# Stanford-ILIAD/PantheonRL

Measured on AMD Instinct MI355X. Metric: env-steps/sec (all agents) Overcooked-simple PPO self-play, higher is better.
Workload: dtype f32; 1 GPU; OvercookedMultiEnv-v0 layout=simple, PPO self-play (two independent PPO learners per GPU), synthetic (n_envs, n_steps, obs_dim) rollouts; n_envs=1024, n_steps=128, obs_dim=62, features=62, n_logits=6, batch_size=32768, n_epochs=10, agents_per_gpu=2, parallelism=2 agent(s) per gpu x1 gpu(s) = 2 learners (single process), launch_mode=graph, gemm_mode=2, action_masks=none, rollout=scripted, rollout_requested=scripted

## Files before the change

### include/pantheon_hip.h

```cpp
#ifndef PANTHEON_HIP_H
#define PANTHEON_HIP_H

#ifdef __cplusplus
extern "C" {
#endif

#define PH_ABI_VERSION 7
#define PH_HIDDEN 64
#define PH_MAX_COMP 256
#define PH_MAX_LOGITS 64
#define PH_MAX_BOX_ACT 16
#define PH_NSTAT 8
#define PH_MOD_MAX 8
#define PH_MAX_RANKS 16

#define PH_SPACE_BOX 0
#define PH_SPACE_DISCRETE 1

typedef struct ph_ctx ph_ctx;

typedef struct ph_space {
  int kind;
  int n;
  int nvec[PH_MAX_COMP];
// ... 8 lines not shown
  int D;
  int F;
  int A;
  int L;
  int P;
  int pi_W1, pi_b1, pi_W2, pi_b2, vf_W1, vf_b1, vf_W2, vf_b2, act_W, act_b, val_W, val_b;
} ph_layout;

typedef struct ph_rollout {
  int T, E;
  float *observations;
  float *actions;
  float *rewards;
  float *episode_starts;
  float *values;
  float *log_probs;
  float *advantages;
  float *returns;
} ph_rollout;

typedef struct ph_ppo_hyper {
  float learning_rate;
  float clip_range;
  float clip_range_vf;
  float ent_coef;
  float vf_coef;
  float max_grad_norm;
  float target_kl;
  int normalize_advantage;
  float adam_beta1, adam_beta2, adam_eps;
} ph_ppo_hyper;

typedef struct ph_opt_state {
  float *params;
  float *adam_m;
  float *adam_v;
  int *step;
} ph_opt_state;

int ph_abi_version(void);
const char *ph_last_error(void);
int ph_device_count(int *n_out );
int ph_ctx_create(int device, ph_ctx **out );
int ph_ctx_destroy(ph_ctx *ctx);
int ph_ctx_set_stream(ph_ctx *ctx, void *hip_stream );
int ph_ctx_sync(ph_ctx *ctx);
int ph_graph_begin(ph_ctx *ctx);
int ph_graph_end(ph_ctx *ctx, int *graph_id_out );
int ph_graph_launch(ph_ctx *ctx, int graph_id);
int ph_ctx_set_rng_epoch(ph_ctx *ctx, unsigned long long *epoch_dev );
int ph_rng_epoch_advance(ph_ctx *ctx);
int ph_debug_set_profile_buffer(ph_ctx *ctx, long long *stamps_dev);
int ph_debug_weight_image_mismatches(ph_ctx *ctx, const ph_spec *spec, const float *params, int *mismatches);
int ph_set_exclusive_device(ph_ctx *ctx, int exclusive);
int ph_ctx_step_errors(ph_ctx *ctx, unsigned int *count_out );
int ph_timer_start(ph_ctx *ctx);
int ph_timer_stop(ph_ctx *ctx, float *ms_out );

int ph_layout_of(const ph_spec *spec , ph_layout *out );
int ph_debug_split_tables(const ph_spec *spec, int *slab_map, int *image_map, int *eligible);
int ph_debug_split_oh_tables(const ph_spec *spec, int *slab_map, int *image_map, int *slab_len_out, int *image_elems_out,
                             int *eligible);

int ph_buffer_add(ph_ctx *ctx, const ph_spec *spec, const ph_rollout *rb, int pos, const float *obs ,
                  const float *actions , const float *episode_start ,
                  const float *values , const float *log_probs );
int ph_buffer_add_reward(ph_ctx *ctx, const ph_rollout *rb, int pos, const float *reward ,
                         const unsigned char *env_mask );
int ph_buffer_add_reward_const(ph_ctx *ctx, const ph_rollout *rb, int pos, float reward);
#define PH_JOINT_MATCH_BONUS 0
#define PH_JOINT_RPS 1
int ph_ctx_set_joint_reward_rule(ph_ctx *ctx, int rule);

int ph_buffer_add_reward_joint(ph_ctx *ctx, const ph_rollout *rb, int pos, const float *base_reward ,
                               const int *joint_actions, int n_seats, int seat, const int *partner_seat ,
                               float bonus);
int ph_roundrobin_env_step(ph_ctx *ctx, const int *joint_actions, int *partnerid, const float *base_reward,
                           const float *done, float *reward_out, int *alt_action_out, float *next_block, int block_ld,
                           int n_partners, float bonus, int n);
typedef struct ph_rr_link {
  int n_partners, rank;
  int n, block_ld;
  void *area[PH_MAX_RANKS];
  unsigned long long *error;
  unsigned long long timeout_cycles;
} ph_rr_link;
typedef struct ph_rr_ego {
  const ph_spec *spec;
  const float *params;
  const float *obs_seq;
  const float *base_reward_seq;
  const float *done_seq;
  float *blocks;
  int *partnerid;
  float *rewards;
  int *alt_actions;
  int *partner_trace;
  const float *episode_start0;
  unsigned long long seed, counter0;
  float *values, *log_probs;
  const ph_rollout *rb;
  float bonus;
} ph_rr_ego;
typedef struct ph_rr_partner {
  const ph_spec *spec;
  const float *params;
// ... 444 lines not shown
```

### pantheonrl_amd/_native.py

```python
from __future__ import annotations

import ctypes as C
import os
from typing import Optional, Sequence

PH_HIDDEN = 64
PH_MAX_COMP = 256
PH_MAX_LOGITS = 64
PH_MAX_BOX_ACT = 16
PH_NSTAT = 8
PH_SPACE_BOX = 0
PH_SPACE_DISCRETE = 1
STAT_NAMES = ("policy_loss", "value_loss", "entropy_loss", "clip_fraction", "approx_kl", "loss", "grad_norm", "applied")

_HERE = os.path.dirname(os.path.abspath(__file__))
LIB_PATH = os.environ.get("PANTHEON_HIP_LIB") or os.path.join(_HERE, "csrc", "libpantheon_hip.so")


class NativeError(RuntimeError):
    """Raised for any non-zero status from the C ABI (message from ph_last_error)."""


class PhSpace(C.Structure):
    _fields_ = [("kind", C.c_int), ("n", C.c_int), ("nvec", C.c_int * PH_MAX_COMP)]
# ... 160 lines not shown
                ("alt_values", C.c_void_p), ("alt_log_probs", C.c_void_p), ("alt_pos", C.c_void_p),
                ("alt_boundary", C.c_void_p), ("alt_term", C.c_void_p), ("alt_open", C.c_void_p), ("alt_acted", C.c_void_p),
                ("alt_seed", C.c_ulonglong),
                ("obs_ego", C.c_void_p), ("obs_alt", C.c_void_p), ("episodes", C.c_void_p),
                ("es_alt", C.c_void_p), ("running", C.c_void_p), ("can", C.c_void_p), ("done", C.c_void_p)]


PH_BLOCK_STATE_WORDS = 12

PH_MAX_POOL = 8
PH_POOL_LEARNER, PH_POOL_FROZEN, PH_POOL_SCRIPTED = 0, 1, 2
POOL_RESAMPLE = {"robin": 0, "random": 1}


class PhPoolMember(C.Structure):
    _fields_ = [("kind", C.c_int), ("params", C.c_void_p), ("rb", C.POINTER(PhRollout)), ("pos", C.c_void_p),
                ("boundary", C.c_void_p), ("term", C.c_void_p), ("open", C.c_void_p), ("values", C.c_void_p),
                ("log_probs", C.c_void_p), ("seed", C.c_ulonglong)]


class PhLiarPool(C.Structure):
    _fields_ = [("n", C.c_int), ("spec", C.POINTER(PhSpec)),
                ("hands", C.c_void_p), ("history", C.c_void_p), ("nmoves", C.c_void_p), ("ego_first", C.c_void_p),
                ("dice_seed", C.c_ulonglong), ("probegostart", C.c_float),
                ("ego_params", C.c_void_p), ("ego_rb", C.POINTER(PhRollout)), ("ego_actions", C.c_void_p),
                ("ego_values", C.c_void_p), ("ego_log_probs", C.c_void_p), ("ego_episode_start", C.c_void_p),
                ("ego_seed", C.c_ulonglong),
                ("members", C.POINTER(PhPoolMember)), ("n_members", C.c_int), ("partnerid", C.c_void_p),
                ("resample", C.c_int), ("pool_seed", C.c_ulonglong),
                ("alt_actions", C.c_void_p), ("alt_acted", C.c_void_p),
                ("obs_ego", C.c_void_p), ("obs_alt", C.c_void_p), ("episodes", C.c_void_p),
                ("obs_next", C.c_void_p), ("rew1", C.c_void_p), ("rew2", C.c_void_p), ("es_alt", C.c_void_p),
                ("done1", C.c_void_p), ("done2", C.c_void_p), ("running", C.c_void_p), ("can", C.c_void_p),
                ("alt_opens", C.c_void_p), ("ego_opens", C.c_void_p), ("done", C.c_void_p)]

SIGNATURES = {
    "ph_abi_version": [],
    "ph_roundrobin_env_step": [_vp, _vp, _vp, _vp, _vp, _vp, _vp, _vp, _i, _i, C.c_float, _i],
    "ph_last_error": [],
    "ph_device_count": [C.POINTER(_i)],
    "ph_ctx_create": [_i, C.POINTER(_vp)],
    "ph_ctx_destroy": [_vp],
    "ph_ctx_set_stream": [_vp, _vp],
    "ph_ctx_sync": [_vp],
    "ph_graph_begin": [_vp],
    "ph_graph_end": [_vp, C.POINTER(_i)],
    "ph_graph_launch": [_vp, _i],
    "ph_ctx_set_rng_epoch": [_vp, _vp],
    "ph_rng_epoch_advance": [_vp],
    "ph_debug_set_profile_buffer": [_vp, _vp],
    "ph_set_exclusive_device": [_vp, _i],
    "ph_ctx_step_errors": [_vp, C.POINTER(C.c_uint)],
    "ph_debug_weight_image_mismatches": [_vp, C.POINTER(PhSpec), _vp, C.POINTER(C.c_int)],
    "ph_timer_start": [_vp],
    "ph_timer_stop": [_vp, C.POINTER(C.c_float)],
    "ph_layout_of": [C.POINTER(PhSpec), C.POINTER(PhLayout)],
    "ph_debug_split_tables": [C.POINTER(PhSpec), C.POINTER(C.c_int), C.POINTER(C.c_int), C.POINTER(C.c_int)],
    "ph_debug_split_oh_tables": [C.POINTER(PhSpec), _vp, _vp, C.POINTER(_i), C.POINTER(_i), C.POINTER(_i)],
    "ph_buffer_add": [_vp, C.POINTER(PhSpec), C.POINTER(PhRollout), _i, _vp, _vp, _vp, _vp, _vp],
    "ph_buffer_add_reward": [_vp, C.POINTER(PhRollout), _i, _vp, _vp],
    "ph_buffer_add_reward_joint": [_vp, C.POINTER(PhRollout), _i, _vp, _vp, _i, _i, _vp, C.c_float],
    "ph_buffer_reset": [_vp, C.POINTER(PhSpec), C.POINTER(PhRollout)],
    "ph_gae": [_vp, C.POINTER(PhRollout), _vp, _vp, _d, _d, _i],
    "ph_policy_forward": [_vp, C.POINTER(PhSpec), _vp, _vp, _i, _vp, _vp, _vp, _ull, _ull, _i, _vp, _vp, _vp, _vp, _vp,
                          _vp, C.POINTER(PhRollout), _i, _vp, _vp, _i],
    "ph_ctx_set_joint_reward_rule": [_vp, _i],
    "ph_adapmult_layout_of": [C.POINTER(PhSpec), _i, _vp],
    "ph_adapmult_forward": [_vp, C.POINTER(PhSpec), _i, _vp, _vp, _i, _vp, _vp, _vp, _ull, _ull, _i, _vp, _vp, _vp, _vp, _vp,
                            _vp, C.POINTER(PhRollout), _i, _vp],
    "ph_adapmult_minibatch_grad": [_vp, C.POINTER(PhSpec), _i, _vp, C.POINTER(PhRollout), C.POINTER(PhPpoHyper), _vp, _i, _vp, _vp,
                                   _vp],
    "ph_adapmult_train": [_vp, C.POINTER(PhSpec), _i, C.POINTER(PhOptState), C.POINTER(PhRollout), C.POINTER(PhPpoHyper), _i, _i,
                          _vp, _ull, _vp, _vp],
    "ph_policy_act_host": [_vp, C.POINTER(PhSpec), _vp, _vp, _i, _vp, _ull, _ull, _i, _vp, _vp, _vp, C.POINTER(PhRollout), _i, _i],
    "ph_buffer_add_reward_const": [_vp, C.POINTER(PhRollout), _i, C.c_float],
    "ph_policy_step_multi": [_vp, _i, C.POINTER(PhStepCall)],
    "ph_policy_forward_ragged": [_vp, C.POINTER(PhSpec), _vp, _vp, _vp, _ull, _ull, _i, _vp, _vp, _vp, C.POINTER(PhRollout),
                                 _vp, _vp, _vp],
    "ph_buffer_add_reward_ragged": [_vp, C.POINTER(PhRollout), _vp, _vp, _vp],
    "ph_ragged_advance": [_vp, C.POINTER(PhRollout), _vp, _vp],
    "ph_buffer_compact_columns": [_vp, C.POINTER(PhSpec), C.POINTER(PhRollout), C.POINTER(PhRollout), _vp, _i],
    "ph_fix_illegal_actions": [_vp, _vp, _vp, _i, _i],
    "ph_rps_step": [_vp, _vp, _vp, _vp, _vp, _i],
    "ph_liar_step": [_vp, _vp, _vp, _vp, _vp, _vp, _vp, _vp, _vp, _vp, _i],
    "ph_liar_reset": [_vp, _vp, _vp, _vp, _vp, _vp, _ull, _ull, C.c_float, _i],
    "ph_liar_obs": [_vp, _vp, _vp, _vp, _vp, _vp, _vp, _i],
    "ph_liar_selfplay_step": [_vp, C.POINTER(PhLiarSelfPlay), _i, _ull, _i],
    "ph_liar_selfplay_rollout": [_vp, C.POINTER(PhLiarSelfPlay), _i, _i, _ull],
    "ph_pool_forward": [_vp, C.POINTER(PhSpec), C.POINTER(PhPoolMember), _i, _vp, _vp, _vp, _ull, _vp, _vp, _i],
    "ph_liar_default_actions": [_vp, _vp, _vp, _vp, _i],
    "ph_liar_pool_step": [_vp, C.POINTER(PhLiarPool), _i, _ull, _i],
    "ph_block_reset": [_vp, _i, _vp, _vp, _ull, _ull, _i],
    "ph_block_step": [_vp, _i, _vp, _vp, _i, _vp, _vp, _vp, _vp, _i],
    "ph_block_obs": [_vp, _i, _vp, _i, _vp, _vp, _i],
    "ph_block_selfplay_step": [_vp, C.POINTER(PhBlockSelfPlay), _i, _ull],
    "ph_block_replay_host": [_i, _i, _i, _vp, _vp, _vp, _vp, _vp, _vp, _vp, _i, _ull, _ull, _i],
    "ph_framestack_push": [_vp, _vp, _vp, _vp, _vp, _i, _i, _i],
    "ph_scripted_rollout": [_vp, C.POINTER(PhSpec), _vp, _vp, _vp, _vp, _i, _i, _vp, _ull, _ull, _vp, _vp, _vp,
                            C.POINTER(PhRollout), _i, _i],
    "ph_ppo_train": [_vp, C.POINTER(PhSpec), C.POINTER(PhOptState), C.POINTER(PhRollout), C.POINTER(PhPpoHyper), _i, _i,
                     _vp, _ull, _vp, _i],
    "ph_ppo_train_multi": [C.POINTER(PhTrainCall), _i],
    "ph_comm_unique_id": [_vp],
    "ph_comm_init": [_vp, _vp, _i, _i],
    "ph_comm_destroy": [_vp],
    "ph_all_gather_i32": [_vp, _vp, _vp, _i],
# ... 114 lines not shown
def make_arch(widths: Sequence[int]) -> PhArch:
    a = PhArch()
    a.n_layers = len(widths)
    for i, w in enumerate(list(widths)[:PH_ARCH_MAX_LAYERS]):
        a.width[i] = int(w)
    return a


def arch_layout_of(spec: PhSpec, arch: PhArch) -> PhArchLayout:
    lay = PhArchLayout()
    check(load().ph_arch_layout_of(C.byref(spec), C.byref(arch), C.byref(lay)))
    return lay


def arch_lds_bytes(spec: PhSpec, arch: PhArch):
    g, r, f = C.c_int(0), C.c_int(0), C.c_int(0)
    check(load().ph_arch_lds_bytes(C.byref(spec), C.byref(arch), C.byref(g), C.byref(r), C.byref(f)))
    return g.value, r.value, f.value


def adapmult_layout_of(spec: PhSpec, context_size: int) -> PhAdapMultLayout:
    lay = PhAdapMultLayout()
    check(load().ph_adapmult_layout_of(C.byref(spec), int(context_size), C.byref(lay)))
    return lay


def ptr(t) -> Optional[int]:
    if t is None:
        return None
    return t.data_ptr()


class Context:

    def __init__(self, device_index: int = 0):
        self.lib = load()
        h = C.c_void_p()
        check(self.lib.ph_ctx_create(int(device_index), C.byref(h)))
        self.handle = h
        self.device_index = int(device_index)
        self.exclusive_hint = False

    def set_stream(self, raw_stream: int) -> None:
        if raw_stream != getattr(self, "_bound_stream", None):
            check(self.lib.ph_ctx_set_stream(self.handle, C.c_void_p(raw_stream)))
            self._bound_stream = raw_stream

    def sync(self) -> None:
        check(self.lib.ph_ctx_sync(self.handle))

    def set_joint_reward_rule(self, rule: str) -> None:
        check(self.lib.ph_ctx_set_joint_reward_rule(self.handle, {"match": 0, "rps": 1}[rule]))

    def step_errors(self) -> int:
        n = C.c_uint(0)
        check(self.lib.ph_ctx_step_errors(self.handle, C.byref(n)))
        return int(n.value)

    def set_exclusive_device(self, exclusive: bool) -> None:
        check(self.lib.ph_set_exclusive_device(self.handle, int(bool(exclusive))))
        self.exclusive_hint = bool(exclusive)

    def close(self) -> None:
        if getattr(self, "handle", None):
            self.lib.ph_ctx_destroy(self.handle)
            self.handle = None

    def __del__(self):
        try:
            self.close()
        except Exception:
            pass


def feistel_indices(n: int, perm_seed: int, epoch: int, start: int = 0, count: Optional[int] = None):
    import numpy as np
    count = n - start if count is None else count
    out = (C.c_int * count)()
    check(load().ph_feistel_indices(int(n), int(perm_seed), int(epoch), int(start), int(count), out))
    return np.frombuffer(out, dtype=np.int32).copy()


def block_replay_host(variant: int, state=None, tokens=None, alt_actions=None, n: Optional[int] = None, seed: Optional[int] = None,
                      counter: int = 0, max_draws: int = -1):
    import numpy as np
    reset = state is None
    if reset:
        state = np.zeros((int(n), PH_BLOCK_STATE_WORDS), np.int32)
    state = np.ascontiguousarray(state, np.int32).copy()
    n = state.shape[0]
    R = 0 if tokens is None else int(np.shape(tokens)[0])
    De, Da, A = ((98, 50, 3) if variant == 1 else (40, 21, 2))
    tok = np.ascontiguousarray(np.zeros((0, n)) if tokens is None else tokens, np.int32).reshape(R, n)
    act = np.ascontiguousarray(np.zeros((0, n, A)) if alt_actions is None else alt_actions, np.int32).reshape(R, n, A)
    alt_obs, ego_obs = np.zeros((R, n, Da), np.float32), np.zeros((R, n, De), np.float32)
    rew, done = np.zeros((R, n, 2), np.float32), np.zeros((R, n), np.uint8)
    p = lambda a: a.ctypes.data_as(C.c_void_p)
    check(load().ph_block_replay_host(int(variant), n, R, p(state), p(tok), p(act), p(alt_obs), p(rew), p(done), p(ego_obs),
                                      int(reset), int(seed or 0), int(counter), int(max_draws)))
    return dict(state=state, alt_obs=alt_obs, rewards=rew, done=done, ego_obs=ego_obs)
```

### pantheonrl_amd/csrc/ph_abi.hip

```cpp
#include <dlfcn.h>
#include <hip/hip_runtime.h>
#include <rccl/rccl.h>

#include <atomic>
#include <chrono>
#include <cmath>
#include <cstdio>
#include <cstdint>
#include <cstring>
#include <mutex>
#include <string>
#include <vector>

#include "ph_launch.h"
#include "ph_block.h"
#include "ph_arch.h"
#include "ph_pool.h"

namespace ph {

namespace {
struct LdsGrant {
  const void* kernel;
  int device;
// ... 62 lines not shown
struct SpecCache {
  ph_spec spec;
  int* obs_off = nullptr;
  int* act_off = nullptr;
  int* slab_map = nullptr;
  int* slab_map_split = nullptr;
  int* wimage_map = nullptr;
  int split_kind = 0;
  int slab_len_split = 0;
  int wimage_elems = 0;
  int id = 0;
};

}

struct ph_ctx {
  int device = 0;
  hipStream_t stream = nullptr;
  float* slabs = nullptr;
  size_t slabs_cap = 0;
  float* statpart = nullptr;
  size_t statpart_cap = 0;
  float* grad = nullptr;
  size_t grad_cap = 0;
  float* blocksq = nullptr;
  size_t blocksq_cap = 0;
  float* advstats = nullptr;
  size_t advstats_cap = 0;
  float* act_stage_host = nullptr;
  float* act_stage_dev = nullptr;
  size_t act_stage_cap = 0;
  unsigned int* act_done_host = nullptr;
  unsigned int* act_done_dev = nullptr;
  unsigned int act_seq = 0;
  unsigned int* fwd_host_done = nullptr;
  int joint_reward_rule = 0;
  int wimage_zeroed_for = 0;
  size_t wimage_cap = 0;
  bool exclusive = false;
  unsigned short* wimage = nullptr;
  double* advpart = nullptr;
  size_t advpart_cap = 0;
  int* perm_idx = nullptr;
  size_t perm_idx_cap = 0;
  int* perm_phys = nullptr;
  size_t perm_phys_cap = 0;
  uint4* ximg = nullptr;
  size_t ximg_cap = 0;
  uint4* rec_pi = nullptr;
  uint4* rec_vf = nullptr;
  size_t rec_cap = 0;
  uint4* rowrec = nullptr;
  size_t rowrec_cap = 0;
  unsigned long long* step_words = nullptr;
  size_t step_words_cap = 0;
  unsigned int* step_gen = nullptr;
  float* am_buf = nullptr;
  size_t am_buf_cap = 0;
  float* adap_extra = nullptr;
  size_t adap_extra_cap = 0;
  float* adap_loss = nullptr;
  size_t adap_loss_cap = 0;
  float* scalars = nullptr;
  int* stop_flag = nullptr;
  std::vector<SpecCache> specs;
  std::vector<hipGraphExec_t> graphs;
  bool capturing = false;
  hipEvent_t ev0 = nullptr, ev1 = nullptr;
  ph_p2p* p2p_dev = nullptr;
  ph_p2p p2p_host;
  bool p2p_valid = false;
  void* comm = nullptr;
  int comm_world = 1, comm_rank = 0;
  hipEvent_t ev_grad = nullptr;
  int num_cu = 256;
  int exchange_blocks_per_cu = 0;
  unsigned long long* rng_epoch = nullptr;
  ph::PoolMemberDev* pool_dev = nullptr;
  ph::PoolMemberDev pool_host[PH_MAX_POOL];
  int pool_count = 0;
  int* pool_order = nullptr;
  size_t pool_order_cap = 0;
  int* pool_tiles = nullptr;
  size_t pool_tiles_cap = 0;
  long long* prof = nullptr;
  struct ModWs {
    float* act = nullptr;
    size_t act_cap = 0;
    int* maps = nullptr;
    ph_spec spec;
    ph_modular mod;
    bool maps_valid = false;
    float* kl_sum = nullptr;
    int* scratch = nullptr;
  } mw;
};

namespace {

struct DevGuard {
  int prev = -1;
  bool switched = false;
  explicit DevGuard(const ph_ctx* ctx) {
    if (!ctx) return;
    if (hipGetDevice(&prev) == hipSuccess && prev != ctx->device) switched = hipSetDevice(ctx->device) == hipSuccess;
  }
  ~DevGuard() {
    if (switched) (void)hipSetDevice(prev);
  }
  DevGuard(const DevGuard&) = delete;
  DevGuard& operator=(const DevGuard&) = delete;
};

template <typename T>
int ensure(const ph_ctx* ctx, T*& p, size_t& cap, size_t n) {
  if (n <= cap) return 0;
  if (ctx->capturing) return fail("workspace would grow inside graph capture: run the same call once outside capture first");
  if (p) (void)hipFree(p);
  p = nullptr;
  cap = 0;
  hipError_t e = hipMalloc((void**)&p, n * sizeof(T));
  if (e != hipSuccess) return fail_hip("hipMalloc(workspace)", e);
  cap = n;
  return 0;
}

int check_space(const ph_space& s, const char* name) {
  if (s.kind != PH_SPACE_BOX && s.kind != PH_SPACE_DISCRETE) return fail(std::string(name) + ": unknown space kind");
  if (s.n <= 0) return fail(std::string(name) + ": empty space");
  if (s.kind == PH_SPACE_DISCRETE) {
    if (s.n > PH_MAX_COMP) return fail(std::string(name) + ": too many components");
    for (int i = 0; i < s.n; ++i)
      if (s.nvec[i] <= 0) return fail(std::string(name) + ": nvec entries must be positive");
  }
  return 0;
}

int layout_of(const ph_spec* spec, ph_layout* o) {
  if (!spec || !o) return fail("null spec/layout");
  if (check_space(spec->obs, "observation space")) return 1;
  if (check_space(spec->act, "action space")) return 1;
  const bool gauss = spec->act.kind == PH_SPACE_BOX;
  if (gauss && spec->act.n > PH_MAX_BOX_ACT) return fail("Box action spaces: at most PH_MAX_BOX_ACT dimensions");
  o->D = spec->obs.n;
  o->F = 0;
  if (spec->obs.kind == PH_SPACE_BOX) o->F = spec->obs.n;
  else
    for (int i = 0; i < spec->obs.n; ++i) o->F += spec->obs.nvec[i];
  o->A = spec->act.n;
  o->L = 0;
  if (gauss) o->L = spec->act.n;
  else
    for (int i = 0; i < spec->act.n; ++i) o->L += spec->act.nvec[i];
  if (o->L > PH_MAX_LOGITS) return fail("too many logits (PH_MAX_LOGITS)");
  const int H = PH_HIDDEN;
  int off = 0;
  o->pi_W1 = off; off += o->F * H;
// ... 239 lines not shown
  ad.nblk = ph::reduce_blocks(slab_len);
  ad.P = P;
  ad.step = opt->step;
  ad.scalars = ctx->scalars;
  ad.stop_flag = ctx->stop_flag;
  ad.lr = hp->learning_rate;
  ad.beta1 = hp->adam_beta1;
  ad.beta2 = hp->adam_beta2;
  ad.eps = hp->adam_eps;
  ad.max_norm = hp->max_grad_norm;
  ad.stats_out = stats_out;
  ad.wimage = wimage;
  ad.wimage_map = wimage_map;
  return ad;
}

int check_train_call(const char* who, const ph_ctx* ctx, const ph_opt_state* opt, const ph_ppo_hyper* hp, int n_epochs,
                     int batch_size, bool aligned = true) {
  const std::string w(who);
  if (!ctx) return fail("null ctx");
  if (!opt || !opt->params || !opt->adam_m || !opt->adam_v || !opt->step) return fail(w + ": null optimizer state");
  if (aligned && (uintptr_t)opt->params % 16 != 0) return fail(w + ": params must be 16-byte aligned");
  if (!hp) return fail(w + ": null hyper-parameters");
  if (n_epochs <= 0 || batch_size <= 0) return fail(w + ": n_epochs and batch_size must be positive");
  return 0;
}
int check_minibatch_call(const char* who, const ph_ctx* ctx, const float* params, const ph_rollout* rb, const ph_ppo_hyper* hp,
                         const int* indices, int nb, const float* grad_out, bool aligned = true) {
  const std::string w(who);
  if (!ctx) return fail("null ctx");
  if (!params || !hp || !indices || !grad_out) return fail(w + ": null argument");
  if (aligned && (uintptr_t)params % 16 != 0) return fail(w + ": params must be 16-byte aligned");
  if (check_rb(rb)) return 1;
  if (nb <= 0) return fail(w + ": nb must be positive");
  return 0;
}

template <typename F>
int time_reps(ph_ctx* ctx, int warm, int reps, F&& fn, float* avg_ms) {
  for (int i = 0; i < warm; ++i)
    if (fn(i)) return 1;
  PH_HIP(hipEventRecord(ctx->ev0, ctx->stream));
  for (int i = 0; i < reps; ++i)
    if (fn(i)) return 1;
  PH_HIP(hipEventRecord(ctx->ev1, ctx->stream));
  PH_HIP(hipEventSynchronize(ctx->ev1));
  float ms = 0.f;
  PH_HIP(hipEventElapsedTime(&ms, ctx->ev0, ctx->ev1));
  *avg_ms = ms / (float)reps;
  return 0;
}
int hip_rc(hipError_t e, const char* what) { return e == hipSuccess ? 0 : fail_hip(what, e); }

}

extern "C" {

int ph_abi_version(void) { return PH_ABI_VERSION; }
const char* ph_last_error(void) { return g_err.c_str(); }

int ph_device_count(int* n_out) {
  if (!n_out) return fail("null n_out");
  int n = 0;
  hipError_t e = hipGetDeviceCount(&n);
  if (e != hipSuccess) {
    *n_out = 0;
    return fail_hip("hipGetDeviceCount", e);
  }
  *n_out = n;
  return 0;
}

int ph_ctx_create(int device, ph_ctx** out) {
  if (!out) return fail("null out");
  *out = nullptr;
  int n = 0;
  hipError_t e = hipGetDeviceCount(&n);
  if (e != hipSuccess || n <= 0) return fail("no HIP device visible: the PantheonRL MI355X engine has no CPU fallback");
  if (device < 0 || device >= n) return fail("device index out of range");
  ph_ctx probe;
  probe.device = device;
  DevGuard dev_guard(&probe);
  hipDeviceProp_t prop;
  PH_HIP(hipGetDeviceProperties(&prop, device));
  if (std::strncmp(prop.gcnArchName, "gfx950", 6) != 0)
    return fail(std::string("device is ") + prop.gcnArchName + ", this library is built for gfx950 (MI355X) only");
  ph_ctx* c = new ph_ctx();
  c->device = device;
  c->num_cu = prop.multiProcessorCount;
  if (hipMalloc((void**)&c->scalars, 4 * sizeof(float)) != hipSuccess ||
      hipMalloc((void**)&c->stop_flag, sizeof(int)) != hipSuccess) {
    delete c;
    return fail("hipMalloc(ctx scalars) failed");
  }
  (void)hipMemset(c->scalars, 0, 4 * sizeof(float));
  (void)hipMemset(c->stop_flag, 0, sizeof(int));
  (void)hipEventCreate(&c->ev0);
  (void)hipEventCreate(&c->ev1);
  *out = c;
  return 0;
}

int ph_ctx_destroy(ph_ctx* ctx) {
  DevGuard dev_guard(ctx);
  if (!ctx) return 0;
  (void)hipStreamSynchronize(ctx->stream);
  for (auto g : ctx->graphs)
    if (g) (void)hipGraphExecDestroy(g);
  for (auto& s : ctx->specs) {
    if (s.obs_off) (void)hipFree(s.obs_off);
    if (s.slab_map) (void)hipFree(s.slab_map);
    if (s.slab_map_split) (void)hipFree(s.slab_map_split);
    if (s.wimage_map) (void)hipFree(s.wimage_map);
    if (s.act_off) (void)hipFree(s.act_off);
  }
  void* ptrs[] = {ctx->wimage, ctx->mw.act, ctx->mw.maps, ctx->mw.kl_sum, ctx->mw.scratch, ctx->advpart, ctx->p2p_dev, ctx->slabs, ctx->statpart, ctx->grad, ctx->blocksq, ctx->advstats, ctx->perm_idx, ctx->perm_phys, ctx->ximg, ctx->rec_pi, ctx->rec_vf, ctx->rowrec, ctx->step_words, ctx->step_gen, ctx->scalars, ctx->stop_flag,
                  ctx->adap_extra, ctx->adap_loss, ctx->am_buf, ctx->pool_dev, ctx->pool_order, ctx->pool_tiles};
  for (void* p : ptrs)
    if (p) (void)hipFree(p);
  if (ctx->act_stage_host) (void)hipHostFree(ctx->act_stage_host);
  if (ctx->act_done_host) (void)hipHostFree(ctx->act_done_host);
  if (ctx->ev0) (void)hipEventDestroy(ctx->ev0);
  if (ctx->ev1) (void)hipEventDestroy(ctx->ev1);
  if (ctx->ev_grad) (void)hipEventDestroy(ctx->ev_grad);
  (void)ph_comm_destroy(ctx);
  delete ctx;
  return 0;
}

int ph_ctx_set_joint_reward_rule(ph_ctx* ctx, int rule) {
  if (!ctx) return fail("null ctx");
  if (rule != PH_JOINT_MATCH_BONUS && rule != PH_JOINT_RPS) return fail("ph_ctx_set_joint_reward_rule: unknown rule");
  ctx->joint_reward_rule = rule;
  return 0;
}

int ph_ctx_set_stream(ph_ctx* ctx, void* hip_stream) {
  DevGuard dev_guard(ctx);
  if (!ctx) return fail("null ctx");
  ctx->stream = (hipStream_t)hip_stream;
  return 0;
}

int ph_ctx_sync(ph_ctx* ctx) {
  DevGuard dev_guard(ctx);
  if (!ctx) return fail("null ctx");
  PH_HIP(hipStreamSynchronize(ctx->stream));
  return 0;
}

int ph_graph_begin(ph_ctx* ctx) {
  DevGuard dev_guard(ctx);
  if (!ctx) return fail("null ctx");
  if (ctx->capturing) return fail("already capturing");
  if (ctx->stream == nullptr) return fail("graph capture needs a non-default stream (ph_ctx_set_stream)");
  PH_HIP(hipStreamBeginCapture(ctx->stream, hipStreamCaptureModeRelaxed));
  ctx->capturing = true;
  return 0;
}

int ph_graph_end(ph_ctx* ctx, int* graph_id_out) {
  DevGuard dev_guard(ctx);
  if (!ctx || !graph_id_out) return fail("null ctx/graph_id_out");
  if (!ctx->capturing) return fail("not capturing");
  ctx->capturing = false;
  hipGraph_t g = nullptr;
  PH_HIP(hipStreamEndCapture(ctx->stream, &g));
  hipGraphExec_t ge = nullptr;
  hipError_t e = hipGraphInstantiate(&ge, g, nullptr, nullptr, 0);
  (void)hipGraphDestroy(g);
  if (e != hipSuccess) return fail_hip("hipGraphInstantiate", e);
  ctx->graphs.push_back(ge);
  *graph_id_out = (int)ctx->graphs.size() - 1;
  return 0;
}

int ph_graph_launch(ph_ctx* ctx, int graph_id) {
  DevGuard dev_guard(ctx);
  if (!ctx) return fail("null ctx");
  if (graph_id < 0 || graph_id >= (int)ctx->graphs.size()) return fail("bad graph id");
  PH_HIP(hipGraphLaunch(ctx->graphs[graph_id], ctx->stream));
  return 0;
}

int ph_ctx_set_rng_epoch(ph_ctx* ctx, unsigned long long* epoch_dev) {
  DevGuard dev_guard(ctx);
  if (!ctx) return fail("null ctx");
  ctx->rng_epoch = epoch_dev;
  return 0;
}
int ph_rng_epoch_advance(ph_ctx* ctx) {
  DevGuard dev_guard(ctx);
  if (!ctx) return fail("null ctx");
  if (!ctx->rng_epoch) return fail("ph_rng_epoch_advance: no epoch word attached");
  PH_HIP(ph::launch_epoch_advance(ctx->rng_epoch, ctx->stream));
  return 0;
}

int ph_debug_set_profile_buffer(ph_ctx* ctx, long long* stamps_dev) {
  DevGuard dev_guard(ctx);
  if (!ctx) return fail("null ctx");
  ctx->prof = stamps_dev;
  return 0;
}

int ph_debug_weight_image_mismatches(ph_ctx* ctx, const ph_spec* spec, const float* params, int* mismatches_host) {
  DevGuard dev_guard(ctx);
  if (!ctx || !params || !mismatches_host) return fail("ph_debug_weight_image_mismatches: null argument");
  ph::NetDims nd;
  if (resolve(ctx, spec, &nd)) return 1;
  *mismatches_host = -1;
  if (!ctx->wimage || !nd.wimage_map) return 0;
  int* d = nullptr;
  PH_HIP(hipMalloc((void**)&d, sizeof(int)));
  PH_HIP(hipMemsetAsync(d, 0, sizeof(int), ctx->stream));
  PH_HIP(ph::launch_weight_image_check(params, ctx->wimage, nd.wimage_map, nd.lay.P, d, ctx->stream));
  PH_HIP(hipMemcpyAsync(mismatches_host, d, sizeof(int), hipMemcpyDeviceToHost, ctx->stream));
  PH_HIP(hipStreamSynchronize(ctx->stream));
  (void)hipFree(d);
  return 0;
}

int ph_set_exclusive_device(ph_ctx* ctx, int exclusive) {
  if (!ctx) return fail("null ctx");
  ctx->exclusive = exclusive != 0;
  return 0;
}

int ph_ctx_step_errors(ph_ctx* ctx, unsigned int* count_out) {
  DevGuard dev_guard(ctx);
  if (!ctx || !count_out) return fail("ph_ctx_step_errors: null argument");
  *count_out = 0u;
  if (!ctx->step_gen) return 0;
  PH_HIP(hipMemcpyAsync(count_out, ctx->step_gen + 1, sizeof(unsigned int), hipMemcpyDeviceToHost, ctx->stream));
  PH_HIP(hipStreamSynchronize(ctx->stream));
  return 0;
}

int ph_timer_start(ph_ctx* ctx) {
  DevGuard dev_guard(ctx);
  if (!ctx) return fail("null ctx");
  PH_HIP(hipEventRecord(ctx->ev0, ctx->stream));
  return 0;
}
int ph_timer_stop(ph_ctx* ctx, float* ms_out) {
  DevGuard dev_guard(ctx);
  if (!ctx || !ms_out) return fail("null ctx/ms_out");
  PH_HIP(hipEventRecord(ctx->ev1, ctx->stream));
  PH_HIP(hipEventSynchronize(ctx->ev1));
  PH_HIP(hipEventElapsedTime(ms_out, ctx->ev0, ctx->ev1));
  return 0;
}

int ph_layout_of(const ph_spec* spec, ph_layout* out) { return layout_of(spec, out); }

int ph_debug_split_tables(const ph_spec* spec, int* slab_map , int* image_map , int* eligible) {
  if (!spec || !slab_map || !image_map || !eligible) return fail("ph_debug_split_tables: null argument");
  ph_layout lay;
  if (layout_of(spec, &lay)) return 1;
  ph::NetDims probe;
  std::memset(&probe, 0, sizeof(probe));
  probe.lay = lay;
  probe.nchunk = (lay.F + PH_HIDDEN - 1) / PH_HIDDEN;
  probe.A = lay.A;
  probe.L = lay.L;
  probe.F = lay.F;
  probe.obs_kind = spec->obs.kind;
  *eligible = ph::grad_split_eligible(probe) ? 1 : 0;
  if (!*eligible) return 0;
  ph::grad_slab_map_split(lay, slab_map, ph::grad_fast_fold(probe));
  ph::grad_weight_image_map(lay, ph::grad_fast_fold(probe), image_map);
  return 0;
}

int ph_debug_split_oh_tables(const ph_spec* spec, int* slab_map, int* image_map , int* slab_len_out, int* image_elems_out,
                             int* eligible) {
  if (!spec || !slab_len_out || !image_elems_out || !eligible) return fail("ph_debug_split_oh_tables: null argument");
  ph_layout lay;
  if (layout_of(spec, &lay)) return 1;
  ph::NetDims probe;
  std::memset(&probe, 0, sizeof(probe));
  probe.lay = lay;
  probe.nchunk = (lay.F + PH_HIDDEN - 1) / PH_HIDDEN;
  probe.A = lay.A;
  probe.L = lay.L;
  probe.F = lay.F;
  probe.D = lay.D;
  probe.obs_kind = spec->obs.kind;
  *eligible = ph::grad_split_oh_eligible(probe) ? 1 : 0;
  if (!*eligible) return 0;
  *slab_len_out = ph::grad_split_oh_slab_len(probe);
  *image_elems_out = ph::grad_split_oh_wimage_elems(probe);
  if (slab_map) ph::grad_slab_map_split_oh(lay, probe.nchunk, slab_map);
  if (image_map) ph::grad_weight_image_map_oh(lay, probe.nchunk, image_map);
  return 0;
}

int ph_buffer_add(ph_ctx* ctx, const ph_spec* spec, const ph_rollout* rb, int pos, const float* obs,
                  const float* actions, const float* episode_start, const float* values, const float* log_probs) {
  DevGuard dev_guard(ctx);
  if (!ctx) return fail("null ctx");
  ph_layout lay;
  if (layout_of(spec, &lay) || check_rb(rb)) return 1;
  if (pos < 0 || pos >= rb->T) return fail("ph_buffer_add: pos out of range (buffer full?)");
  if (!obs || !actions || !episode_start || !values || !log_probs) return fail("ph_buffer_add: null input");
  const size_t E = rb->E, row = (size_t)pos * E;
  PH_HIP(ph::launch_buffer_add(rb->observations + row * lay.D, rb->actions + row * lay.A, rb->rewards + row,
                               rb->episode_starts + row, rb->values + row, rb->log_probs + row, obs, actions,
                               episode_start, values, log_probs, rb->E, lay.D, lay.A, ctx->stream));
  return 0;
}

int ph_buffer_compact_columns(ph_ctx* ctx, const ph_spec* spec, const ph_rollout* src, const ph_rollout* dst,
                              const int* cols, int n) {
  DevGuard dev_guard(ctx);
  if (!ctx) return fail("null ctx");
  ph_layout lay;
  if (layout_of(spec, &lay) || check_rb(src) || check_rb(dst)) return 1;
  if (!cols || n <= 0 || n > src->E) return fail("ph_buffer_compact_columns: bad column list");
  if (dst->T != src->T || dst->E != n) return fail("ph_buffer_compact_columns: destination must be (T, n)");
  PH_HIP(ph::launch_buffer_compact(*src, *dst, cols, n, lay.D, lay.A, ctx->stream));
  return 0;
}

int ph_buffer_add_reward(ph_ctx* ctx, const ph_rollout* rb, int pos, const float* reward,
                         const unsigned char* env_mask) {
  DevGuard dev_guard(ctx);
  if (!ctx) return fail("null ctx");
  if (check_rb(rb)) return 1;
  if (pos < 0 || pos >= rb->T) return fail("ph_buffer_add_reward: pos out of range");
  if (!reward) return fail("ph_buffer_add_reward: null reward");
  PH_HIP(ph::launch_reward_add(rb->rewards + (size_t)pos * rb->E, reward, env_mask, rb->E, ctx->stream));
  return 0;
}

int ph_buffer_add_reward_const(ph_ctx* ctx, const ph_rollout* rb, int pos, float reward) {
  DevGuard dev_guard(ctx);
  if (!ctx) return fail("null ctx");
  if (check_rb(rb)) return 1;
  if (pos < 0 || pos >= rb->T) return fail("ph_buffer_add_reward_const: pos out of range");
  PH_HIP(ph::launch_reward_add_const(rb->rewards + (size_t)pos * rb->E, reward, rb->E, ctx->stream));
  return 0;
}

int ph_buffer_add_reward_joint(ph_ctx* ctx, const ph_rollout* rb, int pos, const float* base_reward,
                               const int* joint_actions, int n_seats, int seat, const int* partner_seat, float bonus) {
  DevGuard dev_guard(ctx);
  if (!ctx) return fail("null ctx");
  if (check_rb(rb)) return 1;
  if (pos < 0 || pos >= rb->T) return fail("ph_buffer_add_reward_joint: pos out of range");
  if (!base_reward || !joint_actions || !partner_seat) return fail("ph_buffer_add_reward_joint: null argument");
  if (n_seats <= 0 || seat < 0 || seat >= n_seats) return fail("ph_buffer_add_reward_joint: bad seat");
  PH_HIP(ph::launch_reward_add_joint(rb->rewards + (size_t)pos * rb->E, base_reward, joint_actions, rb->E, n_seats, seat,
                                     partner_seat, bonus, ctx->joint_reward_rule, ctx->stream));
  return 0;
}

int ph_roundrobin_env_step(ph_ctx* ctx, const int* joint_actions, int* partnerid, const float* base_reward, const float* done,
                           float* reward_out, int* alt_action_out, float* next_block, int block_ld, int n_partners,
                           float bonus, int n) {
  DevGuard dev_guard(ctx);
  if (!ctx) return fail("null ctx");
  if (!joint_actions || !partnerid || !base_reward || !done || !reward_out)
    return fail("ph_roundrobin_env_step: null argument");
  if (n <= 0 || n_partners <= 0) return fail("ph_roundrobin_env_step: bad sizes");
  if (next_block && block_ld < 3) return fail("ph_roundrobin_env_step: routing block rows need >= 3 header columns");
  PH_HIP(ph::launch_roundrobin_env_step(joint_actions, partnerid, base_reward, done, reward_out, alt_action_out, next_block,
                                        block_ld, n_partners, bonus, n, ctx->stream));
  return 0;
}

namespace {
constexpr size_t RR_STAMP_BYTES = 64 * sizeof(unsigned long long);
size_t rr_slot_bytes(int n_partners, int n, int block_ld) {
  const size_t blk = (size_t)n * (block_ld + 1) * sizeof(float), act = (size_t)(n_partners + 1) * n * sizeof(int);
  return ((blk > act ? blk : act) + 255) / 256 * 256;
}
int check_rr_link(const ph_rr_link* l) {
  if (!l) return fail("null ph_rr_link");
  if (l->n_partners < 1 || l->n_partners + 1 > PH_MAX_RANKS) return fail("ph_rr_link: n_partners out of range");
  if (l->rank < 0 || l->rank > l->n_partners || l->n <= 0 || l->block_ld <= 3) return fail("ph_rr_link: bad rank / n / block_ld");
  if (!l->error) return fail("ph_rr_link: error word required");
  for (int r = 0; r <= l->n_partners; ++r)
    if (!l->area[r]) return fail("ph_rr_link: unmapped peer area");
  return 0;
}
unsigned long long* rr_stamps(const ph_rr_link* l, int rank) { return (unsigned long long*)l->area[rank]; }
unsigned int* rr_arrive(const ph_rr_link* l) { return (unsigned int*)((unsigned long long*)l->area[0] + 32); }
char* rr_slot(const ph_rr_link* l, int rank, int parity) {
  return (char*)l->area[rank] + RR_STAMP_BYTES + (size_t)parity * rr_slot_bytes(l->n_partners, l->n, l->block_ld);
}
}

int ph_rr_area_bytes(int n_partners, int n, int block_ld, size_t* bytes_out) {
  if (!bytes_out || n_partners < 1 || n <= 0 || block_ld <= 3) return fail("ph_rr_area_bytes: bad argument");
  *bytes_out = RR_STAMP_BYTES + 2 * rr_slot_bytes(n_partners, n, block_ld);
  return 0;
}

int ph_roundrobin_ego_iteration(ph_ctx* ctx, const ph_rr_link* link, const ph_rr_ego* ego, int T, unsigned long long iteration) {
// ... 63 lines not shown
    return fail("ph_roundrobin_partner_iteration: null argument");
  if (check_rb(pa->rb)) return 1;
  if (pa->rb->E != link->n) return fail("ph_roundrobin_partner_iteration: the rollout buffer must have one column per environment");
  const int n = link->n, k = link->rank - 1;
  for (int t = 0; t < T; ++t) {
    const unsigned long long want = iteration * (unsigned long long)T + (unsigned long long)t + 1ull;
    ph::RRPartnerStep st;
    std::memset(&st, 0, sizeof(st));
    st.block_stamp = rr_stamps(link, link->rank);
    st.act_stamp = rr_stamps(link, 0) + 1 + k;
    st.want = want;
    st.timeout = link->timeout_cycles;
    st.error = link->error;
    st.block = (const float*)rr_slot(link, link->rank, t & 1);
    st.block_ld = link->block_ld;
    st.n = n;
    st.T = pa->rb->T;
    st.k = k;
    st.rewards = pa->rb->rewards;
    st.pos = pa->pos;
    st.boundary = pa->boundary;
    st.term = pa->term;
    st.open = pa->open;
    st.prev_mask = pa->prev_mask;
    st.can = pa->can_scratch;
    st.es = pa->es_scratch;
    st.actions = pa->actions;
    st.act_dst = (int*)rr_slot(link, 0, t & 1) + (size_t)(1 + k) * n;
    PH_HIP(ph::launch_rr_partner_pre(st, ctx->stream));
    const float* obs_t = st.block + (size_t)n * 4;
    if (ph_policy_forward_ragged(ctx, pa->spec, pa->params, obs_t, nullptr, pa->seed, pa->counter0 + (unsigned long long)t,
                                 0, pa->actions, pa->values, pa->log_probs, pa->rb, pa->pos, pa->can_scratch, pa->es_scratch))
      return 1;
    PH_HIP(ph::launch_rr_partner_post(st, ctx->stream));
  }
  return 0;
}

int ph_buffer_reset(ph_ctx* ctx, const ph_spec* spec, const ph_rollout* rb) {
  DevGuard dev_guard(ctx);
  if (!ctx) return fail("null ctx");
  ph_layout lay;
  if (layout_of(spec, &lay) || check_rb(rb)) return 1;
  const size_t n = (size_t)rb->T * rb->E;
  PH_HIP(hipMemsetAsync(rb->observations, 0, n * lay.D * sizeof(float), ctx->stream));
  PH_HIP(hipMemsetAsync(rb->actions, 0, n * lay.A * sizeof(float), ctx->stream));
  float* arrs[] = {rb->rewards, rb->episode_starts, rb->values, rb->log_probs, rb->advantages, rb->returns};
  for (float* a : arrs) PH_HIP(hipMemsetAsync(a, 0, n * sizeof(float), ctx->stream));
  return 0;
}

int ph_gae(ph_ctx* ctx, const ph_rollout* rb, const float* last_values, const float* dones, double gamma,
           double gae_lambda, int mode) {
  DevGuard dev_guard(ctx);
  if (!ctx) return fail("null ctx");
  if (check_rb(rb)) return 1;
  if (!last_values || !dones) return fail("ph_gae: null last_values/dones");
  if (mode < 0 || mode > 2) return fail("ph_gae: mode must be 0, 1 or 2");
  PH_HIP(ph::launch_gae(rb->rewards, rb->values, rb->episode_starts, last_values, dones, rb->advantages, rb->returns,
                        rb->T, rb->E, gamma, gae_lambda, mode, ctx->stream));
  return 0;
}

int ph_policy_forward(ph_ctx* ctx, const ph_spec* spec, const float* params, const float* obs, int n,
                      const unsigned char* action_mask, const float* uniforms, const float* given_actions,
                      unsigned long long seed, unsigned long long counter, int deterministic, int* actions_i32,
                      float* actions_f32, float* values, float* log_probs, float* entropy, float* logits,
                      const ph_rollout* rb, int pos, const float* episode_start_in, const float* pending_reward,
                      int gemm_mode) {
  DevGuard dev_guard(ctx);
  if (!ctx) return fail("null ctx");
  if (!params || !obs) return fail("ph_policy_forward: null params/obs");
  if ((uintptr_t)params % 16 != 0) return fail("ph_policy_forward: params must be 16-byte aligned");
  if (n <= 0) return fail("ph_policy_forward: n must be positive");
  ph::FwdArgs a;
  if (fwd_args(a, ctx, spec, true, params, obs, n, seed, counter, actions_i32, values, log_probs)) return 1;
  if (a.nd.gauss && action_mask) return fail("ph_policy_forward: action masks belong to the categorical heads");
  a.mask = action_mask;
  a.uniforms = uniforms;
  a.given_actions = given_actions;
  a.prof = ctx->prof;
  a.deterministic = deterministic;
  a.act_f32 = actions_f32;
  a.entropy = entropy;
  a.logits = logits;
  if (fwd_bind_row("ph_policy_forward", a, rb, pos, episode_start_in, pending_reward)) return 1;
  a.host_done = ctx->fwd_host_done;
  a.host_seq = ctx->act_seq;
  PH_HIP(ph::launch_policy_fwd(a, gemm_mode, ctx->stream));
  return 0;
}

int ph_policy_act_host(ph_ctx* ctx, const ph_spec* spec, const float* params, const float* obs_host, int n,
                       const float* episode_start_host, unsigned long long seed, unsigned long long counter, int deterministic,
                       int* actions_host, float* values_host, float* log_probs_host, const ph_rollout* rb, int pos, int gemm_mode) {
  DevGuard dev_guard(ctx);
  if (!ctx) return fail("null ctx");
  if (!params || !obs_host) return fail("ph_policy_act_host: null params/obs");
  if (n <= 0) return fail("ph_policy_act_host: n must be positive");
  if (rb && !episode_start_host) return fail("ph_policy_act_host: the fused rollout-buffer write needs episode_start_host");
  if (ctx->capturing) return fail("ph_policy_act_host synchronises: not inside graph capture");
  ph::NetDims nd;
  if (resolve(ctx, spec, &nd)) return 1;
  const size_t n_in = (size_t)n * nd.D + (size_t)n, n_out = (size_t)n * nd.A + 2 * (size_t)n, need = n_in + n_out;
  if (need > ctx->act_stage_cap) {
    if (ctx->act_stage_host) (void)hipHostFree(ctx->act_stage_host);
    ctx->act_stage_host = nullptr;
    ctx->act_stage_dev = nullptr;
    ctx->act_stage_cap = 0;
    const size_t cap = need < 4096 ? 4096 : need;
    PH_HIP(hipHostMalloc((void**)&ctx->act_stage_host, cap * sizeof(float), hipHostMallocMapped | hipHostMallocCoherent));
    PH_HIP(hipHostGetDevicePointer((void**)&ctx->act_stage_dev, ctx->act_stage_host, 0));
    ctx->act_stage_cap = cap;
  }
  float *h = ctx->act_stage_host, *d = ctx->act_stage_dev;
  std::memcpy(h, obs_host, (size_t)n * nd.D * sizeof(float));
  if (episode_start_host) std::memcpy(h + (size_t)n * nd.D, episode_start_host, (size_t)n * sizeof(float));
  else std::memset(h + (size_t)n * nd.D, 0, (size_t)n * sizeof(float));
  float* d_out = d + n_in;
  int* d_act = reinterpret_cast<int*>(d_out);
  float *d_val = d_out + (size_t)n * nd.A, *d_lp = d_val + n;
  const bool words = n <= 16 && ph::fwd16_eligible(nd, n);
  if (words && !ctx->act_done_host) {
    PH_HIP(hipHostMalloc((void**)&ctx->act_done_host, 64, hipHostMallocMapped | hipHostMallocCoherent));
    PH_HIP(hipHostGetDevicePointer((void**)&ctx->act_done_dev, ctx->act_done_host, 0));
    ctx->act_done_host[0] = ctx->act_done_host[1] = 0;
  }
  if (words) {
    if (++ctx->act_seq == 0) ctx->act_seq = 1;
    ctx->fwd_host_done = ctx->act_done_dev;
  }
  const int frc = ph_policy_forward(ctx, spec, params, d, n, nullptr, nullptr, nullptr, seed, counter, deterministic, d_act,
                                    nullptr, d_val, d_lp, nullptr, nullptr, rb, pos, rb ? d + (size_t)n * nd.D : nullptr, nullptr,
                                    gemm_mode);
  ctx->fwd_host_done = nullptr;
  if (frc) return 1;
  bool arrived = false;
  if (words) {
    const unsigned int seq = ctx->act_seq;
    const auto t0 = std::chrono::steady_clock::now();
    for (unsigned spins = 0;; ++spins) {
      if (__atomic_load_n(ctx->act_done_host, __ATOMIC_ACQUIRE) == seq &&
          __atomic_load_n(ctx->act_done_host + 1, __ATOMIC_ACQUIRE) == seq) {
        arrived = true;
        break;
      }
      if ((spins & 1023) == 1023 && std::chrono::steady_clock::now() - t0 > std::chrono::milliseconds(50)) break;
      __builtin_ia32_pause();
    }
  }
  if (!arrived) PH_HIP(hipStreamSynchronize(ctx->stream));
  const float* h_out = h + n_in;
  if (actions_host) std::memcpy(actions_host, h_out, (size_t)n * nd.A * sizeof(int));
  if (values_host) std::memcpy(values_host, h_out + (size_t)n * nd.A, (size_t)n * sizeof(float));
  if (log_probs_host) std::memcpy(log_probs_host, h_out + (size_t)n * nd.A + n, (size_t)n * sizeof(float));
  return 0;
}

int ph_scripted_rollout(ph_ctx* ctx, const ph_spec* spec, const float* params, const float* obs_seq, const float* rew_seq,
                        const float* done_seq, int n, int n_steps, const float* episode_start0, unsigned long long seed,
                        unsigned long long counter0, int* actions_i32, float* values, float* log_probs, const ph_rollout* rb,
                        int pos0, int gemm_mode) {
  DevGuard dev_guard(ctx);
  if (!ctx) return fail("null ctx");
  if (!params || !obs_seq || !rew_seq || !done_seq || !episode_start0) return fail("ph_scripted_rollout: null argument");
  if ((uintptr_t)params % 16 != 0) return fail("ph_scripted_rollout: params must be 16-byte aligned");
  if (n <= 0 || n_steps <= 0) return fail("ph_scripted_rollout: n and n_steps must be positive");
  if (check_rb(rb)) return 1;
  if (n != rb->E) return fail("ph_scripted_rollout: n must equal the rollout buffer's E");
  if (pos0 < 0 || pos0 + n_steps > rb->T) return fail("ph_scripted_rollout: rows pos0 .. pos0 + n_steps - 1 must lie in the buffer");
  ph::FwdArgs a;
  if (fwd_args(a, ctx, spec, false, params, obs_seq, n, seed, counter0, actions_i32, values, log_probs)) return 1;
  if (!ph::fwd16_eligible(a.nd, n))
    return fail("ph_scripted_rollout: needs the 16-row forward's shape class (one feature chunk, one Discrete head of <= 8 logits, "
                "n < 16384); use ph_policy_forward per step");
  a.prof = ctx->prof;
  if (fwd_bind_row("ph_scripted_rollout", a, rb, pos0, episode_start0, nullptr)) return 1;
  ph::ScriptedSteps sc;
  sc.n_steps = n_steps;
  sc.obs_seq = obs_seq;
  sc.rew_seq = rew_seq;
  sc.done_seq = done_seq;
  sc.mask_seq = nullptr;
  PH_HIP(ph::launch_policy_fwd16_rollout(a, sc, gemm_mode, ctx->stream));
  return 0;
}

namespace {
int step_multi_impl(ph_ctx* ctx, int n_calls, const ph_step_call* calls, const ph_p2p* x, int t);
int ensure_p2p_dev(ph_ctx* ctx, const ph_p2p* x);
}
int ph_policy_step_multi(ph_ctx* ctx, int n_calls, const ph_step_call* calls) {
  DevGuard dev_guard(ctx);
  return step_multi_impl(ctx, n_calls, calls, nullptr, 0);
}
namespace {
int step_multi_impl(ph_ctx* ctx, int n_calls, const ph_step_call* calls, const ph_p2p* x, int t) {
  if (!ctx) return fail("null ctx");
  if (!calls) return fail("ph_policy_step_multi: null calls");
  if (n_calls <= 0 || n_calls > ph::MAX_LOCAL_AGENTS) return fail("ph_policy_step_multi: 1..4 calls per launch");
  ph::FwdMulti m;
  std::memset(&m, 0, sizeof(m));
  for (int i = 0; i < n_calls; ++i) {
    const ph_step_call& c = calls[i];
    ph::FwdArgs& a = m.a[i];
    if (!c.params || !c.obs || !c.rb || !c.episode_start_in) return fail("ph_policy_step_multi: null argument");
    if ((uintptr_t)c.params % 16 != 0) return fail("ph_policy_step_multi: params must be 16-byte aligned");
    if (fwd_args(a, ctx, c.spec, false, c.params, c.obs, c.n, c.seed, c.counter, c.actions_i32, c.values, c.log_probs)) return 1;
    if (fwd_bind_row("ph_policy_step_multi", a, c.rb, c.pos, c.episode_start_in, c.pending_reward)) return 1;
    if (i > 0 && (c.n != calls[0].n || a.nd.Lp != m.a[0].nd.Lp))
      return fail("ph_policy_step_multi: all calls must share n and the padded logit count");
    a.mask = c.action_mask;
    a.deterministic = c.deterministic & 1;
    if (c.deterministic & (PH_STEP_FIX_ILLEGAL | PH_STEP_MASK_ENV_ONLY)) {
      if (!c.action_mask) return fail("PH_STEP_FIX_ILLEGAL / PH_STEP_MASK_ENV_ONLY need an action mask");
      if (!(a.nd.A == 1 && a.nd.L <= 8))
        return fail("PH_STEP_FIX_ILLEGAL: single Discrete head of at most 8 logits only (use ph_fix_illegal_actions)");
      a.env_mask = c.action_mask;
      if (c.deterministic & PH_STEP_MASK_ENV_ONLY) a.mask = nullptr;
    }
    if (c.pending_reward && c.joint_actions) {
      if (!c.partner_seat || c.n_seats <= 0 || c.seat < 0 || c.seat >= c.n_seats)
        return fail("ph_policy_step_multi: bad joint-action description");
      a.joint = c.joint_actions;
      a.n_seats = c.n_seats;
      a.seat = c.seat;
      a.partner_seat = c.partner_seat;
      a.bonus = c.bonus;
      a.reward_rule = ctx->joint_reward_rule;
    }
  }
  if (x) {
    if (!ph::fwd16_eligible(m.a[0].nd, m.a[0].n)) return fail("fused peer-to-peer step needs the 16-row forward kernel");
    if (x->count != n_calls * m.a[0].n) return fail("ph_p2p.count must be local agents x n");
    if (ensure_p2p_dev(ctx, x)) return 1;
    m.px.x = ctx->p2p_dev;
    m.px.t = t;
// ... 822 lines not shown
    return fail("ph_arch: observation space too large for the tower kernels' LDS tile (" +
                std::to_string(ph::arch_grad_lds_bytes(*nd, *ad, ph::ARCH_FWD_ROWS)) + " bytes at 32 rows, 163840 available)");
  return 0;
}

void fill_grad_args(ph::GradArgs& g, const ph::NetDims& nd, const float* params, const ph_rollout* rb,
                    const ph_ppo_hyper* hp, ph_ctx* ctx) {
  g.nd = nd;
  g.params = params;
  g.rb_obs = rb->observations;
  g.rb_act = rb->actions;
  g.rb_val = rb->values;
  g.rb_logp = rb->log_probs;
  g.rb_adv = rb->advantages;
  g.rb_ret = rb->returns;
  g.T = rb->T;
  g.E = rb->E;
  g.clip = hp->clip_range;
  g.clip_vf = hp->clip_range_vf;
  g.ent_coef = hp->ent_coef;
  g.vf_coef = hp->vf_coef;
  g.norm_adv = hp->normalize_advantage;
  g.slabs = ctx->slabs;
  g.statpart = ctx->statpart;
  g.stop_flag = ctx->stop_flag;
  g.prof = ctx->prof;
  g.wimage = ctx->wimage;
  g.ximg = ctx->ximg;
  g.ximg_zero_row = rb->T * rb->E;
  g.rec_pi = ctx->rec_pi;
  g.rec_vf = ctx->rec_vf;
}

int rebuild_weight_image(ph_ctx* ctx, const ph::NetDims& nd, const float* params) {
  if (!nd.split) return 0;
  if ((size_t)nd.wimage_elems > ctx->wimage_cap) {
    if (ctx->capturing) return fail("first split-kernel use inside graph capture: call it once outside capture first");
    if (ensure(ctx, ctx->wimage, ctx->wimage_cap, (size_t)nd.wimage_elems)) return 1;
    ctx->wimage_zeroed_for = 0;
  }
  if (ctx->wimage_zeroed_for != nd.spec_id) {
    if (ctx->capturing) return fail("the weight image changes its spec inside graph capture: run the same call once outside capture first");
    PH_HIP(hipMemsetAsync(ctx->wimage, 0, (size_t)nd.wimage_elems * sizeof(unsigned short), ctx->stream));
    ctx->wimage_zeroed_for = nd.spec_id;
  }
  PH_HIP(ph::launch_weight_image(params, ctx->wimage, nd.wimage_map, nd.lay.P, ctx->stream));
  return 0;
}

int build_grad_pack(ph_ctx* ctx, const ph::NetDims& nd, const ph_rollout* rb, size_t n_rec) {
  if (nd.split != 1) return 0;
  const size_t rows = (size_t)rb->T * rb->E;
  const size_t need_img = (rows + 1) * ph::XIMG_ROW_U4;
  if (ensure(ctx, ctx->ximg, ctx->ximg_cap, need_img)) return 1;
  if (ensure(ctx, ctx->rowrec, ctx->rowrec_cap, 2 * rows)) return 1;
  if (n_rec > ctx->rec_cap) {
    size_t c1 = ctx->rec_cap, c2 = ctx->rec_cap;
    if (ensure(ctx, ctx->rec_pi, c1, n_rec)) return 1;
    if (ensure(ctx, ctx->rec_vf, c2, n_rec)) return 1;
    ctx->rec_cap = n_rec;
  }
  PH_HIP(ph::launch_obs_planes(rb->observations, (int)rows, nd.D, nd.F, ph::grad_fast_fold(nd) ? 1 : 0, ctx->ximg, rb->advantages,
                               rb->log_probs, rb->actions, rb->returns, rb->values, ctx->rowrec, ctx->stream));
  return 0;
}
void fill_adv_records(ph::AdvStatArgs& aa, const ph_ctx* ctx, const ph::NetDims& nd, const ph_rollout* rb) {
  aa.rec_pi_out = nd.split == 1 ? ctx->rec_pi : nullptr;
  aa.rec_vf_out = nd.split == 1 ? ctx->rec_vf : nullptr;
  aa.rowrec = (nd.split == 1 && rb->advantages && rb->log_probs && rb->actions && rb->returns && rb->values) ? ctx->rowrec : nullptr;
  aa.rb_logp = rb->log_probs;
  aa.rb_act = rb->actions;
  aa.rb_ret = rb->returns;
  aa.rb_val = rb->values;
}


void select_gemm(ph::NetDims& nd, int gemm_mode) {
  nd.split = (gemm_mode == 2 && nd.slab_map_split != nullptr) ? nd.split_kind : 0;
  if (nd.split) nd.slab_map = nd.slab_map_split;
}

int slab_len_of(const ph::NetDims& nd) { return nd.split ? nd.slab_len_split : (nd.slab_map ? 2 * ph::RS_NET : nd.lay.P); }

int ensure_train_ws(ph_ctx* ctx, int P, int slab_len, int nwg_max, int n_mb_total, size_t n_idx = 0, size_t n_phys = 0) {
  if (n_phys && ensure(ctx, ctx->perm_phys, ctx->perm_phys_cap, n_phys)) return 1;
  if (ensure(ctx, ctx->slabs, ctx->slabs_cap, (size_t)nwg_max * slab_len)) return 1;
  if (ensure(ctx, ctx->statpart, ctx->statpart_cap, (size_t)2 * nwg_max * ph::NSTATP)) return 1;
  if (ensure(ctx, ctx->grad, ctx->grad_cap, (size_t)P)) return 1;
  if (ensure(ctx, ctx->blocksq, ctx->blocksq_cap, (size_t)ph::reduce_blocks(slab_len))) return 1;
  if (ensure(ctx, ctx->advstats, ctx->advstats_cap, (size_t)n_mb_total * 2)) return 1;
  if (ensure(ctx, ctx->advpart, ctx->advpart_cap, (size_t)n_mb_total * 2 * ph::ADV_SPLIT)) return 1;
  if (n_idx && ensure(ctx, ctx->perm_idx, ctx->perm_idx_cap, n_idx)) return 1;
  const size_t n_words = (size_t)ph::reduce_blocks(slab_len) + 1;
  if (n_words > ctx->step_words_cap) {
    if (ensure(ctx, ctx->step_words, ctx->step_words_cap, n_words)) return 1;
    PH_HIP(hipMemsetAsync(ctx->step_words, 0, n_words * sizeof(unsigned long long), ctx->stream));
  }
  if (!ctx->step_gen) {
    if (ctx->capturing) return fail("workspace would grow inside graph capture: run the same call once outside capture first");
    PH_HIP(hipMalloc((void**)&ctx->step_gen, 4 * sizeof(unsigned int)));
    PH_HIP(hipMemsetAsync(ctx->step_gen, 0, 4 * sizeof(unsigned int), ctx->stream));
  }
  return 0;
}

bool step_fused_wanted(const ph_ctx* ctx, int slab_len, bool alone) {
  return alone && ctx->exclusive && ctx->step_words && ctx->step_gen &&
         ph::step_fused_fits(ph::reduce_blocks(slab_len), slab_len, ctx->num_cu);
}

}

namespace {

struct TrainPlan {
  int alone = 1;
// ... 153 lines not shown
}

void fill_step_args(const TrainPlan& t, int mbi, const MbPlan& pl, ph::ReduceArgs& r, ph::AdamArgs& ad) {
  ph_ctx* ctx = t.ctx;
  float* stats_out = t.stats ? t.stats + (size_t)mbi * PH_NSTAT : nullptr;
  r = reduce_args(ctx, t.hp, t.opt, t.P, slab_len_of(t.nd), t.nd.slab_map, pl.nwg, pl.nb, ctx->grad, stats_out);
  r.wide = t.alone && ctx->exclusive;
  ad = adam_args(ctx, t.hp, t.opt, t.P, slab_len_of(t.nd), stats_out, t.nd.split ? ctx->wimage : nullptr, t.nd.wimage_map);
}

int train_launch_step(const TrainPlan& t, int mbi, const MbPlan& pl) {
  ph_ctx* ctx = t.ctx;
  hipStream_t s = ctx->stream;
  ph::ReduceArgs r;
  ph::AdamArgs ad;
  fill_step_args(t, mbi, pl, r, ad);
  if (t.adap) {
    const MbWalk w = minibatch_walk(ctx, t.perms, t.N, t.n_mb, t.batch_size, mbi);
    if (adap_launch(ctx, t.nd, t.opt->params, t.rb, t.adap, w.idx, w.nb, mbi, &r)) return 1;
  }
  if (step_fused_wanted(ctx, slab_len_of(t.nd), t.alone != 0)) {
    PH_HIP(ph::launch_ppo_step(r, ad, ctx->step_words, ctx->step_gen, ctx->step_gen + 1, STEP_WAIT_TICKS, s));
  } else {
    PH_HIP(ph::launch_ppo_reduce(r, s));
    PH_HIP(ph::launch_ppo_adam(ad, s));
  }
  return 0;
}

}

namespace {
int train_run(const char* who, ph_ctx* ctx, const ph_spec* spec, const ph_opt_state* opt, const ph_rollout* rb,
              const ph_ppo_hyper* hp, int n_epochs, int batch_size, const int* perms, unsigned long long perm_seed, float* stats,
              int gemm_mode, const ph_adap_loss* adap, const ph_arch* arch = nullptr) {
  TrainPlan t;
  if (train_prepare(who, t, ctx, spec, opt, rb, hp, n_epochs, batch_size, perms, perm_seed, stats, gemm_mode, adap != nullptr, arch))
    return 1;
  if (adap && t.nd.gauss) return fail("ph_adap_train: the context term is written for the categorical heads");
  if (adap && adap_check(ctx, t.nd, adap, "ph_adap_train")) return 1;
  t.adap = adap;
  for (int mbi = 0; mbi < n_epochs * t.n_mb; ++mbi) {
    MbPlan pl;
    if (train_launch_grad(t, mbi, &pl)) return 1;
    if (train_launch_step(t, mbi, pl)) return 1;
  }
  return 0;
}
}

int ph_ppo_train(ph_ctx* ctx, const ph_spec* spec, const ph_opt_state* opt, const ph_rollout* rb,
                 const ph_ppo_hyper* hp, int n_epochs, int batch_size, const int* perms,
                 unsigned long long perm_seed, float* stats, int gemm_mode) {
  DevGuard dev_guard(ctx);
  return train_run("ph_ppo_train", ctx, spec, opt, rb, hp, n_epochs, batch_size, perms, perm_seed, stats, gemm_mode, nullptr);
}

int ph_adap_train(ph_ctx* ctx, const ph_spec* spec, const ph_opt_state* opt, const ph_rollout* rb,
                  const ph_ppo_hyper* hp, int n_epochs, int batch_size, const int* perms,
                  unsigned long long perm_seed, float* stats, int gemm_mode, const ph_adap_loss* adap) {
  DevGuard dev_guard(ctx);
  if (!adap) return fail("ph_adap_train: null context-term description");
  return train_run("ph_adap_train", ctx, spec, opt, rb, hp, n_epochs, batch_size, perms, perm_seed, stats, gemm_mode, adap);
}

int ph_ppo_train_multi(const ph_train_call* calls, int n_calls) {
  if (!calls || n_calls <= 0) return fail("ph_ppo_train_multi: no calls");
  if (n_calls > PH_MAX_TRAIN_CALLS) return fail("ph_ppo_train_multi: too many calls");
  TrainPlan t[PH_MAX_TRAIN_CALLS];
  int total[PH_MAX_TRAIN_CALLS], longest = 0;
  for (int k = 0; k < n_calls; ++k) {
    const ph_train_call& c = calls[k];
    if (train_prepare("ph_ppo_train_multi", t[k], c.ctx, c.spec, c.opt, c.rb, c.hyper, c.n_epochs, c.batch_size, c.perms,
                      c.perm_seed, c.stats, c.gemm_mode))
      return 1;
    t[k].alone = n_calls == 1;
    if (!t[k].ctx->ev_grad) PH_HIP(hipEventCreateWithFlags(&t[k].ctx->ev_grad, hipEventDisableTiming));
    total[k] = c.n_epochs * t[k].n_mb;
    longest = total[k] > longest ? total[k] : longest;
  }
  hipEvent_t prev = nullptr;
  hipStream_t prev_stream = nullptr;
  for (int mbi = 0; mbi < longest; ++mbi) {
    for (int k = 0; k < n_calls; ++k) {
      if (mbi >= total[k]) continue;
      hipStream_t s = t[k].ctx->stream;
      if (prev && prev_stream != s) PH_HIP(hipStreamWaitEvent(s, prev, 0));
      MbPlan pl;
      if (train_launch_grad(t[k], mbi, &pl)) return 1;
      PH_HIP(hipEventRecord(t[k].ctx->ev_grad, s));
      prev = t[k].ctx->ev_grad;
      prev_stream = s;
      if (train_launch_step(t[k], mbi, pl)) return 1;
    }
  }
  return 0;
}

namespace {
int minibatch_grad_run(const char* who, ph_ctx* ctx, const ph_spec* spec, const float* params, const ph_rollout* rb,
                       const ph_ppo_hyper* hp, const int* indices, int nb, float* grad_out, float* stats_out, int gemm_mode,
                       const ph_adap_loss* adap, const ph_arch* arch = nullptr);
}

int ph_ppo_minibatch_grad(ph_ctx* ctx, const ph_spec* spec, const float* params, const ph_rollout* rb,
                          const ph_ppo_hyper* hp, const int* indices, int nb, float* grad_out, float* stats_out,
                          int gemm_mode) {
  DevGuard dev_guard(ctx);
  return minibatch_grad_run("ph_ppo_minibatch_grad", ctx, spec, params, rb, hp, indices, nb, grad_out, stats_out, gemm_mode, nullptr);
}

int ph_adap_minibatch_grad(ph_ctx* ctx, const ph_spec* spec, const float* params, const ph_rollout* rb,
                           const ph_ppo_hyper* hp, const int* indices, int nb, float* grad_out, float* stats_out,
                           int gemm_mode, const ph_adap_loss* adap) {
  DevGuard dev_guard(ctx);
  if (!adap) return fail("ph_adap_minibatch_grad: null context-term description");
  return minibatch_grad_run("ph_adap_minibatch_grad", ctx, spec, params, rb, hp, indices, nb, grad_out, stats_out, gemm_mode, adap);
}

namespace {
int minibatch_grad_run(const char* who, ph_ctx* ctx, const ph_spec* spec, const float* params, const ph_rollout* rb,
                       const ph_ppo_hyper* hp, const int* indices, int nb, float* grad_out, float* stats_out, int gemm_mode,
                       const ph_adap_loss* adap, const ph_arch* arch) {
  if (check_minibatch_call(who, ctx, params, rb, hp, indices, nb, grad_out)) return 1;
  ph::NetDims nd;
  ph::ArchDims ad;
  if (arch) {
    if (arch_resolve(ctx, spec, arch, &nd, &ad)) return 1;
  } else {
    if (resolve(ctx, spec, &nd, adap == nullptr)) return 1;
    select_gemm(nd, gemm_mode);
  }
  const int P = nd.lay.P;
  const MbPlan pl = plan_minibatch(ctx, nd, nb, arch ? &ad : nullptr);
  if (ensure_train_ws(ctx, P, slab_len_of(nd), pl.nwg, 1, 0, (size_t)nb)) return 1;
  hipStream_t s = ctx->stream;
  PH_HIP(ph::launch_set_int(ctx->stop_flag, 0, s));
  if (rebuild_weight_image(ctx, nd, params)) return 1;
  if (build_grad_pack(ctx, nd, rb, (size_t)nb)) return 1;
  ph::AdvStatArgs aa = adv_args_minibatch(ctx, rb, indices, nb);
  fill_adv_records(aa, ctx, nd, rb);
  PH_HIP(ph::launch_adv_stats(aa, 1, s));
  ph::GradArgs g;
  std::memset(&g, 0, sizeof(g));
  fill_grad_args(g, nd, params, rb, hp, ctx);
  g.idx = indices;
  g.idx_phys = ctx->perm_phys;
  g.nb = nb;
  g.advstats = ctx->advstats;
  g.ntiles = pl.ntiles;
  if (arch) PH_HIP(ph::launch_arch_grad(g, ad, pl.nwg, gemm_mode, s));
  else PH_HIP(ph::launch_ppo_grad(g, pl.nwg, gemm_mode, s));
  ph::ReduceArgs r = reduce_args(ctx, hp, nullptr, P, slab_len_of(nd), nd.slab_map, pl.nwg, nb, grad_out, stats_out);
  if (adap) {
    if (adap_check(ctx, nd, adap, who)) return 1;
    if (adap_launch(ctx, nd, params, rb, adap, indices, nb, 0, &r)) return 1;
  }
  PH_HIP(ph::launch_ppo_reduce(r, s));
  return 0;
}
}

int ph_arch_layout_of(const ph_spec* spec, const ph_arch* arch, ph_arch_layout* out) { return arch_layout(spec, arch, out); }

int ph_arch_lds_bytes(const ph_spec* spec, const ph_arch* arch, int* grad_bytes_out, int* grad_rows_out, int* fwd_bytes_out) {
  ph::ArchDims ad;
  std::memset(&ad, 0, sizeof(ad));
  if (arch_layout(spec, arch, &ad.lay)) return 1;
// ... 928 lines not shown
```

### pantheonrl_amd/csrc/ph_gae.hip

```cpp
#include "ph_launch.h"

namespace ph {

__global__ __launch_bounds__(64) void gae_serial_kernel(const float* __restrict__ rew, const float* __restrict__ val,
                                                        const float* __restrict__ es, const float* __restrict__ last_values,
                                                        const float* __restrict__ dones, float* __restrict__ adv,
                                                        float* __restrict__ ret, int T, int E, float g, float gl) {
#pragma clang fp contract(off)
  const int e = blockIdx.x * blockDim.x + threadIdx.x;
  if (e >= E) return;
  float nv = last_values[e];
  float nnt = 1.0f - dones[e];
  float last = 0.f;
  int t = T - 1;
  for (; t >= 7; t -= 8) {
    float r[8], v[8], s[8];
#pragma unroll
    for (int u = 0; u < 8; ++u) {
      const size_t o = (size_t)(t - u) * E + e;
      r[u] = rew[o];
      v[u] = val[o];
      s[u] = es[o];
    }
#pragma unroll
    for (int u = 0; u < 8; ++u) {
      const size_t o = (size_t)(t - u) * E + e;
      const float delta = (r[u] + (g * nv) * nnt) - v[u];
      last = delta + ((gl * nnt) * last);
      adv[o] = last;
      ret[o] = last + v[u];
      nv = v[u];
      nnt = 1.0f - s[u];
    }
  }
  for (; t >= 0; --t) {
    const size_t o = (size_t)t * E + e;
    const float r = rew[o], v = val[o], s = es[o];
    const float delta = (r + (g * nv) * nnt) - v;
    last = delta + ((gl * nnt) * last);
    adv[o] = last;
    ret[o] = last + v;
    nv = v;
    nnt = 1.0f - s;
  }
}

__device__ __forceinline__ float gae_ld(const float* p) { return __builtin_nontemporal_load(p); }
__device__ __forceinline__ void gae_st(float* p, float v) { __builtin_nontemporal_store(v, p); }

template <int LC, int EB>
__global__ __launch_bounds__(1024) void gae_scan_kernel(const float* __restrict__ rew, const float* __restrict__ val,
                                                        const float* __restrict__ es,
                                                        const float* __restrict__ last_values,
                                                        const float* __restrict__ dones, float* __restrict__ adv,
                                                        float* __restrict__ ret, int T, int E, int NCH, float g,
                                                        float gl) {
  extern __shared__ __attribute__((aligned(16))) float sm[];
  float* sS = sm;
  float* sP = sm + NCH * EB;
  float* carry = sP + NCH * EB;
  const int el = threadIdx.x % EB, ch = threadIdx.x / EB;
  const int e = blockIdx.x * EB + el;
  const bool env_ok = e < E;
  const int span = NCH * LC;
  if (ch == 0) carry[el] = 0.f;
  for (int top = T; top > 0; top -= span) {
    const int base = top - span;
    const int t0 = base + ch * LC;
    const int tend = t0 + LC;
    const bool live = env_ok && tend > 0;
    float a[LC], cp[LC], vv[LC];
    float S = 0.f, P = 1.f;
    if (live) {
      float nv, nnt;
      if (tend == T) {
        nv = last_values[e];
        nnt = 1.0f - dones[e];
      } else {
        nv = val[(size_t)tend * E + e];
        nnt = 1.0f - es[(size_t)tend * E + e];
      }
      float r[LC], s[LC];
#pragma unroll
      for (int k = 0; k < LC; ++k) {
        const int t = t0 + k;
        const size_t o = (size_t)(t >= 0 ? t : 0) * E + e;
        r[k] = gae_ld(rew + o);
        vv[k] = gae_ld(val + o);
        s[k] = gae_ld(es + o);
      }
      float A = 0.f, Pacc = 1.f;
#pragma unroll
      for (int k = LC - 1; k >= 0; --k) {
        if (t0 + k >= 0) {
          const float delta = r[k] + g * nv * nnt - vv[k];
          const float c = gl * nnt;
          A = delta + c * A;
          Pacc = c * Pacc;
          nv = vv[k];
          nnt = 1.0f - s[k];
        }
        a[k] = A;
        cp[k] = Pacc;
      }
      S = A;
      P = Pacc;
    }
    __syncthreads();
    sS[ch * EB + el] = S;
    sP[ch * EB + el] = P;
    for (int d = 1; d < NCH; d <<= 1) {
      __syncthreads();
      float S2 = 0.f, P2 = 1.f;
      const bool has = (ch + d < NCH);
      if (has) {
        S2 = sS[(ch + d) * EB + el];
        P2 = sP[(ch + d) * EB + el];
      }
      __syncthreads();
      if (has) {
        S = S + P * S2;
        P = P * P2;
        sS[ch * EB + el] = S;
        sP[ch * EB + el] = P;
      }
    }
    __syncthreads();
    const float cin = carry[el];
    const float Ain = (ch + 1 < NCH) ? sS[(ch + 1) * EB + el] + sP[(ch + 1) * EB + el] * cin : cin;
    const float Afirst = sS[el] + sP[el] * cin;
    __syncthreads();
    if (ch == 0) carry[el] = Afirst;
    if (live) {
#pragma unroll
      for (int k = 0; k < LC; ++k) {
        const int t = t0 + k;
        if (t >= 0) {
          const size_t o = (size_t)t * E + e;
          const float A = a[k] + cp[k] * Ain;
          gae_st(adv + o, A);
          gae_st(ret + o, A + vv[k]);
        }
      }
    }
  }
}

template <int LC, int EB>
static hipError_t launch_scan(const float* rew, const float* val, const float* es, const float* lv, const float* dn,
                              float* adv, float* ret, int T, int E, float g, float gl, hipStream_t s, int max_chunks = 1024 / EB) {
  int NCH = (T + LC - 1) / LC;
  int maxch = max_chunks < 1024 / EB ? max_chunks : 1024 / EB;
  static int nch_env = -1;
  if (nch_env < 0) {
    const char* e = getenv("PH_GAE_NCH");
    nch_env = e ? atoi(e) : 0;
  }
  if (nch_env > 0 && nch_env < maxch) maxch = nch_env;
  if (NCH > maxch) NCH = maxch;
  dim3 grid((E + EB - 1) / EB), block(NCH * EB);
  const size_t lds = sizeof(float) * (2 * NCH * EB + EB);
  hipLaunchKernelGGL((gae_scan_kernel<LC, EB>), grid, block, lds, s, rew, val, es, lv, dn, adv, ret, T, E, NCH, g, gl);
  return hipGetLastError();
}

hipError_t launch_gae(const float* rew, const float* val, const float* es, const float* lv, const float* dn, float* adv,
                      float* ret, int T, int E, double gamma, double lam, int mode, hipStream_t s) {
  const float g = (float)gamma;
  const float gl = (float)(gamma * lam);
  if (mode == 0) mode = 2;
  if (mode == 1) {
    hipLaunchKernelGGL(gae_serial_kernel, dim3((E + 63) / 64), dim3(64), 0, s, rew, val, es, lv, dn, adv, ret, T, E, g,
                       gl);
    return hipGetLastError();
  }
  static int lc_env = -1;
  if (lc_env < 0) {
    const char* e = getenv("PH_GAE_LC");
    lc_env = e ? atoi(e) : 0;
  }
  if (lc_env == 8) return launch_scan<8, 32>(rew, val, es, lv, dn, adv, ret, T, E, g, gl, s);
  if (lc_env == 16) return launch_scan<16, 32>(rew, val, es, lv, dn, adv, ret, T, E, g, gl, s);
  if (lc_env == 32) return launch_scan<32, 32>(rew, val, es, lv, dn, adv, ret, T, E, g, gl, s);
  if (T <= 256) return launch_scan<8, 32>(rew, val, es, lv, dn, adv, ret, T, E, g, gl, s);
  if (E >= 16384) return launch_scan<16, 64>(rew, val, es, lv, dn, adv, ret, T, E, g, gl, s, 16);
  return launch_scan<16, 32>(rew, val, es, lv, dn, adv, ret, T, E, g, gl, s, 8);
}

__global__ void buffer_add_kernel(float* __restrict__ d_obs, float* __restrict__ d_act, float* __restrict__ d_rew,
                                  float* __restrict__ d_es, float* __restrict__ d_val, float* __restrict__ d_lp,
                                  const float* __restrict__ obs, const float* __restrict__ act,
                                  const float* __restrict__ es, const float* __restrict__ val,
                                  const float* __restrict__ lp, int E, int D, int A) {
  const int stride = gridDim.x * blockDim.x;
  const int g0 = blockIdx.x * blockDim.x + threadIdx.x;
  for (int i = g0; i < E * D; i += stride) d_obs[i] = obs[i];
  for (int i = g0; i < E * A; i += stride) d_act[i] = act[i];
  for (int i = g0; i < E; i += stride) {
    d_rew[i] = 0.f;
    d_es[i] = es[i];
    d_val[i] = val[i];
    d_lp[i] = lp[i];
  }
}
hipError_t launch_buffer_add(float* d_obs, float* d_act, float* d_rew, float* d_es, float* d_val, float* d_lp,
                             const float* obs, const float* act, const float* es, const float* val, const float* lp,
                             int E, int D, int A, hipStream_t s) {
  const int n = E * D;
  int blocks = (n + 255) / 256;
  if (blocks > 2048) blocks = 2048;
  if (blocks < 1) blocks = 1;
  hipLaunchKernelGGL(buffer_add_kernel, dim3(blocks), dim3(256), 0, s, d_obs, d_act, d_rew, d_es, d_val, d_lp, obs, act,
                     es, val, lp, E, D, A);
  return hipGetLastError();
}

struct CompactArgs {
  ph_rollout src, dst;
  const int* cols;
  int n, D, A;
};
__global__ void buffer_compact_kernel(CompactArgs a) {
  const int T = a.src.T, E = a.src.E, n = a.n;
  const size_t stride = (size_t)gridDim.x * blockDim.x, g0 = (size_t)blockIdx.x * blockDim.x + threadIdx.x;
  for (size_t i = g0; i < (size_t)T * n * a.D; i += stride) {
    const size_t row = i / a.D, f = i - row * a.D, t = row / n, c = row - t * n;
    a.dst.observations[i] = a.src.observations[(t * E + a.cols[c]) * a.D + f];
  }
  for (size_t i = g0; i < (size_t)T * n * a.A; i += stride) {
    const size_t row = i / a.A, f = i - row * a.A, t = row / n, c = row - t * n;
    a.dst.actions[i] = a.src.actions[(t * E + a.cols[c]) * a.A + f];
  }
  for (size_t i = g0; i < (size_t)T * n; i += stride) {
    const size_t t = i / n, c = i - t * n, j = t * E + a.cols[c];
    a.dst.rewards[i] = a.src.rewards[j];
    a.dst.episode_starts[i] = a.src.episode_starts[j];
    a.dst.values[i] = a.src.values[j];
    a.dst.log_probs[i] = a.src.log_probs[j];
    a.dst.advantages[i] = a.src.advantages[j];
// ... 85 lines not shown
```

### pantheonrl_amd/csrc/ph_launch.h

```cpp
#pragma once
#include "ph_device.h"

namespace ph {

__host__ __device__ inline unsigned p2p_stamp32(unsigned long long epoch, int T, int t) {
  return (unsigned)(epoch * (unsigned long long)T + (unsigned long long)t + 1ull);
}

__device__ __forceinline__ void p2p_note_timeout(unsigned long long* error, int kind, int t, unsigned long long index,
                                                 unsigned long long want, unsigned long long seen) {
  if (atomicAdd(error, 1ull) == 0ull) {
    error[1] = (unsigned long long)(unsigned)kind | ((unsigned long long)(unsigned)(t & 0xffffff) << 8) | (index << 32);
    error[2] = want;
    error[3] = seen;
  }
}

__device__ __forceinline__ void poll_backoff(int& polls) {
  if (polls < 16) __builtin_amdgcn_s_sleep(2);
  else if (polls < 64) __builtin_amdgcn_s_sleep(16);
  else __builtin_amdgcn_s_sleep(127);
  ++polls;
}

// ... 2 lines not shown

struct FwdArgs {
  NetDims nd;
  const float* params;
  const float* obs;
  int n;
  const unsigned char* mask;
  const float* uniforms;
  const float* given_actions;
  uint64_t seed, counter;
  const unsigned long long* epoch;
  int deterministic;
  int* act_i32;
  float* act_f32;
  float* values;
  float* logp;
  float* entropy;
  float* logits;
  float* rb_obs;
  float* rb_act;
  float* rb_rew;
  float* rb_es;
  float* rb_val;
  float* rb_logp;
  const float* es_in;
  long long* prof;
  float* prev_rew;
  const float* pending_reward;
  const int* pos_env;
  const unsigned char* rec_mask;
  int rb_T;
  const int* joint;
  const unsigned long long* joint_ll;
  const unsigned long long* ll_epoch;
  int ll_T, ll_t;
  unsigned long long ll_timeout;
  unsigned long long* ll_error;
  int n_seats, seat;
  const int* partner_seat;
  float bonus;
  int reward_rule;
  const unsigned char* env_mask;
  unsigned int* host_done;
  unsigned int host_seq;
};

struct ScriptedSteps {
  int n_steps;
  const float* obs_seq;
  const float* rew_seq;
  const float* done_seq;
  const unsigned char* mask_seq;
  int mask_policy, mask_env;
};

constexpr int MAX_LOCAL_AGENTS = 4;
struct P2PStep {
  const ph_p2p* x;
  int t;
  int a_local;
  int persistent;
};
__host__ __device__ inline int p2p_persistent_slot(unsigned long long epoch, int T, int t) { return (int)(epoch & 1ull) * T + t; }
struct FwdMulti {
  FwdArgs a[MAX_LOCAL_AGENTS];
  P2PStep px;
};
struct ScriptedMulti {
  ScriptedSteps sc[MAX_LOCAL_AGENTS];
};
bool fwd16_eligible(const NetDims& nd, int n);
hipError_t launch_policy_fwd16_rollout(const FwdArgs& a, const ScriptedSteps& sc, int gemm_mode, hipStream_t s);
hipError_t launch_policy_fwd16_exchange_rollout(const FwdMulti& m, const ScriptedMulti& sm, int n_agents, hipStream_t s);
hipError_t exchange_rollout_blocks_per_cu(int* blocks_out);

struct GradArgs {
  NetDims nd;
  const float* params;
  const float* rb_obs;
  const float* rb_act;
  const float* rb_val;
  const float* rb_logp;
  const float* rb_adv;
  const float* rb_ret;
  int T, E;
  const int* idx;
  const int* idx_phys;
  uint32_t perm_n, perm_hb;
  uint64_t perm_seed;
  int perm_epoch;
  const unsigned long long* epoch;
  int mb_start;
  int nb;
  const float* advstats;
  float clip, clip_vf, ent_coef, vf_coef;
  int norm_adv;
  float* slabs;
  float* statpart;
  const int* stop_flag;
  long long* prof;
  int ntiles;
  const unsigned short* wimage;
  const uint4* ximg;
  int ximg_zero_row;
  const uint4* rec_pi;
  const uint4* rec_vf;
// ... 55 lines not shown
  int nslab, P;
  int slab_len;
  const int* map;
  float* grad;
  float* blocksq;
  const float* statpart;
  int nstatpart;
  float* stats_out;
  int nb;
  float ent_coef, vf_coef, target_kl;
  int* stop_flag;
  int* step;
  float* scalars;
  const float* extra = nullptr;
  int n_extra = 0, extra_len = 0, extra_cut = 0, extra_lo = 0, extra_hi = 0;
  const float* extra_loss = nullptr;
  float extra_norm = 0.f;
  float extra_coef = 0.f;
  float* extra_loss_out = nullptr;
  int wide = 0;
};

struct AdamArgs {
  float* params;
  float* m;
  float* v;
  const float* grad;
  const float* blocksq;
  int nblk, P;
  const int* step;
  const float* scalars;
  int* stop_flag;
  float lr, beta1, beta2, eps, max_norm;
  float* stats_out;
  unsigned short* wimage;
  const int* wimage_map;
};

struct StepArgs {
  ReduceArgs r;
  AdamArgs ad;
  unsigned long long* words = nullptr;
  unsigned int* gen = nullptr;
  unsigned long long timeout = 0;
  unsigned int* sweep_error = nullptr;
};

size_t fwd_lds_bytes(int R, int Lp);
size_t grad_lds_bytes(int R, int Lp, int onehot_D, int nchunk);
hipError_t launch_policy_fwd(const FwdArgs& a, int gemm_mode, hipStream_t s);
hipError_t launch_policy_fwd_multi(const FwdMulti& m, int n_agents, hipStream_t s);
hipError_t launch_fix_illegal(int* actions, const unsigned char* mask, int n, int L, hipStream_t s);
hipError_t launch_gae(const float* rew, const float* val, const float* es, const float* lv, const float* dn, float* adv,
                      float* ret, int T, int E, double gamma, double lam, int mode, hipStream_t s);
hipError_t launch_buffer_add(float* d_obs, float* d_act, float* d_rew, float* d_es, float* d_val, float* d_lp,
                             const float* obs, const float* act, const float* es, const float* val, const float* lp,
                             int E, int D, int A, hipStream_t s);
hipError_t launch_buffer_compact(const ph_rollout& src, const ph_rollout& dst, const int* cols, int n, int D, int A,
                                 hipStream_t s);
hipError_t launch_reward_add_ragged(float* rewards, const int* pos_env, const float* reward, const unsigned char* mask,
                                    int T, int E, hipStream_t s);
hipError_t launch_ragged_advance(int* pos_env, const unsigned char* mask, int T, int E, hipStream_t s);
hipError_t launch_liar_obs(const int* hands, const int* history, const int* nmoves, const unsigned char* is_ego,
                           const unsigned char* active, float* obs_out, int n, hipStream_t s);
hipError_t launch_liar_reset(int* hands, int* history, int* nmoves, const unsigned char* reset_mask,
                             unsigned char* ego_first, unsigned long long seed, unsigned long long counter,
                             const unsigned long long* epoch, float probegostart, int n, hipStream_t s);
hipError_t launch_reward_add(float* rew_row, const float* reward, const unsigned char* env_mask, int E, hipStream_t s);
hipError_t launch_reward_add_const(float* rew_row, float reward, int E, hipStream_t s);
hipError_t launch_reward_add_joint(float* rew_row, const float* base, const int* joint, int E, int n_seats, int seat,
                                   const int* partner_seat, float bonus, int rule, hipStream_t s);
hipError_t launch_framestack_push(float* stack, const float* obs, const unsigned char* reset_mask,
                                  const float* default_obs, int n, int D, int nf, hipStream_t s);
hipError_t launch_roundrobin_env_step(const int* joint, int* partnerid, const float* base, const float* done, float* reward_out,
                                      int* alt_action_out, float* next_block, int block_ld, int n_partners, float bonus, int n,
                                      hipStream_t s);
hipError_t launch_rps_step(const int* ego_act, const int* alt_act, float* ego_rew, float* alt_rew, int n, hipStream_t s);
hipError_t launch_liar_step(const int* hands, int* history, int* nmoves, const int* actions, const unsigned char* is_ego,
                            const unsigned char* active, float* obs_next, float* rew, unsigned char* done, int n,
                            hipStream_t s);
hipError_t launch_ppo_grad(const GradArgs& a, int nwg, int gemm_mode, hipStream_t s);
hipError_t launch_liar_sp_after_ego(const ph_liar_selfplay& s, hipStream_t st);
hipError_t launch_liar_sp_after_reply(const ph_liar_selfplay& s, float* ego_rew_row, unsigned long long counter,
                                      const unsigned long long* epoch, int deal_only, hipStream_t st);
hipError_t launch_liar_sp_after_opening(const ph_liar_selfplay& s, hipStream_t st);
bool liar_rollout_eligible(const NetDims& nd, int n);

constexpr int ADAP_ROWS = 16;
struct AdapArgs {
  NetDims nd;
  const float* params;
  const float* rb_obs;
  int T, E;
  const int* idx;
  int nb;
  int ctx_size, n_ctx, n_states;
  int sampler;
  float coef;
  const int* state_idx;
  const float* contexts;
  uint64_t seed;
  const unsigned long long* epoch;
  uint32_t mbi, nb_hb;
  float* extra;
  float* loss_part;
  int* used_state_idx;
  float* used_contexts;
// ... 63 lines not shown
  const unsigned long long* stamps;
  unsigned long long want, timeout;
  unsigned long long* error;
  const int* joint;
  int* partnerid;
  int* partner_trace;
  const float* base;
  const float* done;
  float* reward_out;
  int* alt_action_out;
  float* next_block;
  int block_ld, n_partners, n;
  float bonus;
};
struct RRPartnerStep {
  const unsigned long long* block_stamp;
  unsigned long long* act_stamp;
  unsigned long long want, timeout;
  unsigned long long* error;
  const float* block;
  int block_ld, n, T, k;
  float* rewards;
  int* pos;
  unsigned char *boundary, *term, *open, *prev_mask, *can;
  float* es;
  const int* actions;
  int* act_dst;
};
hipError_t launch_rr_send_block(const RRSend& a, int n_partners, hipStream_t s);
hipError_t launch_rr_env_step(const RREnvStep& a, hipStream_t s);
hipError_t launch_rr_partner_pre(const RRPartnerStep& a, hipStream_t s);
hipError_t launch_rr_partner_post(const RRPartnerStep& a, hipStream_t s);
constexpr int RS_NET = 8960;
constexpr int RS_W2 = 0, RS_W1 = 4096, RS_B1 = 8192, RS_B2 = 8256, RS_HW = 8320, RS_HB = 8832;
bool grad_fast_eligible(const NetDims& nd);
bool grad_uses_reg_slabs(const NetDims& nd);
bool grad_fast_fold(const NetDims& nd);
void grad_slab_map(const ph_layout& lay, int* map , bool fold);
void grad_plan(const NetDims& nd, int nb, int num_cu, int* ntiles, int* nwg);
hipError_t launch_ppo_grad_fast(const GradArgs& a, int nwg, int gemm_mode, hipStream_t s);
bool grad_split_eligible(const NetDims& nd);
constexpr int WIMG_PLANE = 64 * 8;
constexpr int WIMG_ELEMS = 2 * 4 * 3 * 2 * 3 * WIMG_PLANE;
void grad_weight_image_map(const ph_layout& lay, bool fold, int* map );
hipError_t launch_weight_image(const float* params, unsigned short* image, const int* map, int P, hipStream_t s);
hipError_t launch_weight_image_check(const float* params, const unsigned short* image, const int* map, int P, int* mismatches,
                                     hipStream_t s);
void grad_slab_map_split(const ph_layout& lay, int* map , bool fold);
hipError_t launch_ppo_grad_split(const GradArgs& a, int nwg, hipStream_t s);
hipError_t launch_adv_stats(const AdvStatArgs& a, int n_total, hipStream_t s);
constexpr int XIMG_ROW_U4 = 24;
hipError_t launch_obs_planes(const float* obs, int n, int D, int F, int fold, uint4* image, const float* adv, const float* logp,
                             const float* act, const float* ret, const float* val, uint4* rowrec, hipStream_t s);
hipError_t launch_ppo_reduce(const ReduceArgs& a, hipStream_t s);
int reduce_blocks(int slab_len);
bool step_fused_fits(int nblk, int slab_len, int num_cu);
hipError_t launch_ppo_step(const ReduceArgs& r, const AdamArgs& ad, unsigned long long* words, unsigned int* gen,
                           unsigned int* sweep_error, unsigned long long timeout, hipStream_t st);
hipError_t launch_ppo_adam(const AdamArgs& a, hipStream_t s);
bool grad_split_oh_eligible(const NetDims& nd);
int grad_split_oh_slab_len(const NetDims& nd);
int grad_split_oh_wimage_elems(const NetDims& nd);
void grad_weight_image_map_oh(const ph_layout& lay, int nch, int* map );
void grad_slab_map_split_oh(const ph_layout& lay, int nch, int* map );
hipError_t launch_ppo_grad_split_oh(const GradArgs& a, int nwg, hipStream_t s);
hipError_t launch_set_int(int* p, int v, hipStream_t s);
size_t bc_train_lds_bytes(int F, int L, int P, int A);
hipError_t launch_bc_train(const NetDims& nd, const ph_bc_layout& lay, float* params, float* adam_m, float* adam_v, int* step,
                           const float* obs, const float* acts, const int* order, int N, int batch, int n_epochs,
                           int max_batches, const ph_bc_hyper& hp, float* stats, hipStream_t s);
hipError_t launch_bc_forward(const NetDims& nd, const ph_bc_layout& lay, const float* params, const float* obs, int n,
                             const unsigned char* mask, const float* uniforms, const float* given, uint64_t seed,
                             uint64_t counter, int deterministic, int* act_i32, float* values, float* logp, float* entropy,
                             float* logits, hipStream_t s);
hipError_t launch_epoch_advance(unsigned long long* p, hipStream_t s);

struct TowerArgs {
  int nb, ntiles;
  const float* x;
  int x_ld;
  int F;
  const int* obs_off;
  const int* idx;
  int T, E;
  const float *W1, *b1, *W2, *b2, *hW, *hb;
  int head;
  int L;
  float* h2_out;
  float* head_out;
  const float* dhead;
  const float* ext0;
  const float* ext1;
  float* dx_out;
  int dx_accumulate;
  float* slab;
  int slab_stride;
};
struct TowerLaunch {
  TowerArgs t[2];
  int mode;
  const int* stop_flag;
};
size_t tower_lds_bytes();
hipError_t launch_tower(const TowerLaunch& L, int nwg, int n_towers, int gemm_mode, hipStream_t s);
void tower_slab_map(int F, int L, int head, int oW1, int oB1, int oW2, int oB2, int oHW, int oHB, int* map );

// ... 51 lines not shown
```

### pantheonrl_amd/csrc/ph_policy.hip

```cpp
#include <cstring>
#include <initializer_list>
#include "ph_rowtail.h"
#include "ph_liar_group.h"
#include "ph_pool.h"

namespace ph {


template <int R, int LP, bool VALU>
__device__ __forceinline__ void policy_fwd_body(const FwdArgs& a) {
  extern __shared__ __attribute__((aligned(16))) float smem[];
  constexpr int NT = R * 4;
  const NetDims& nd = a.nd;
  constexpr int Lp = LP, LDO = LP + 1;
  float* bufA = smem;
  float* bufB = bufA + R * LDH;
  float* w1s = bufB + R * LDH;
  float* w2s = w1s + HID * LDH;
  float* wos = w2s + HID * LDH;
  float* outs = wos + HID * LDO;
  float* b1s = outs + R * LDO;
  float* b2s = b1s + HID;
  float* bos = b2s + HID;
  int* rowphys = (int*)(bos + 64);

  const int tid = threadIdx.x;
  const int wave = tid >> 6, lane = tid & 63, li = lane & 31, lh = lane >> 5;
  const int mt = wave >> 1, nt = wave & 1;
  const int net = blockIdx.y;
  const int row0 = blockIdx.x * R;
  const ph_layout& lay = nd.lay;
  const float* W1 = a.params + (net == 0 ? lay.pi_W1 : lay.vf_W1);
  const float* B1 = a.params + (net == 0 ? lay.pi_b1 : lay.vf_b1);
  const float* W2 = a.params + (net == 0 ? lay.pi_W2 : lay.vf_W2);
  const float* B2 = a.params + (net == 0 ? lay.pi_b2 : lay.vf_b2);

  PH_STAMP(a.prof, 0);
  if (tid < R) rowphys[tid] = (row0 + tid < a.n) ? row0 + tid : -1;
  WStage<NT> w2r, w1r;
  WoStage<NT> wor;
  XStage<R, NT> xr;
  w2r.issue(W2, 0, HID);
  w1r.issue(W1, 0, nd.F);
  if (net == 0) wor.issue(a.params + lay.act_W, nd.L, Lp);
  float bias1 = 0.f, bias2 = 0.f, bias3 = 0.f;
  if (tid < HID) {
    bias1 = B1[tid];
    bias2 = B2[tid];
    bias3 = (net == 0) ? ((tid < nd.L) ? a.params[lay.act_b + tid] : 0.f) : a.params[lay.val_W + tid];
  }
  PH_STAMP(a.prof, 8);
  __syncthreads();
  PH_STAMP(a.prof, 9);
  xr.issue(rowphys, a.obs, nd, 0);
  w2r.commit(w2s);
  PH_STAMP(a.prof, 10);
  w1r.commit(w1s);
// ... 58 lines not shown
      f32x16 acc3 = {0};
      acc3 = tile_mma<false, false, VALU>(bufA, LDH, wos, LDO, hm * 32, hn * 32, 0, HID, acc3);
#pragma unroll
      for (int r = 0; r < 16; ++r) {
        const int row = hm * 32 + drow(r, lh), col = hn * 32 + li;
        outs[row * LDO + col] = acc3[r] + bos[col];
      }
    }
  }
  __syncthreads();
  PH_STAMP(a.prof, 6);

  if (tid < R && rowphys[tid] >= 0) general_row_tail(a, nd, row0 + tid, outs + tid * LDO, fwd_counter(a));
  PH_STAMP(a.prof, 7);
}


__device__ __forceinline__ void lds_only_barrier() { asm volatile("s_waitcnt lgkmcnt(0)\n\ts_barrier" ::: "memory"); }
__device__ __forceinline__ void vm_drain() { __builtin_amdgcn_s_waitcnt(0x0F70); }

struct RowStage3 {
  static constexpr int ITERS = 6;
  static constexpr unsigned NONE = 0x80000000u;
  float v[ITERS] = {0.f, 0.f, 0.f, 0.f, 0.f, 0.f};
  __device__ __forceinline__ static unsigned base_offset(int row0, const NetDims& nd, int tid) {
    const int kk = tid & 63, w = (tid >> 6) - 1;
    return (w >= 0 && kk < nd.D && kk < nd.F) ? ((unsigned)(row0 + w) * (unsigned)nd.D + (unsigned)kk) * 4u : NONE;
  }
  __device__ __forceinline__ static unsigned slot_offset(unsigned base, int i, int D, int tid) {
    return (i == 5 && (tid >> 6) != 1) ? NONE : base + (unsigned)(3 * i) * (unsigned)D * 4u;
  }
  __device__ __forceinline__ static __amdgpu_buffer_rsrc_t block(const float* blk, int n, int D) {
    return __builtin_amdgcn_make_buffer_rsrc(const_cast<float*>(blk), 0, n * D * 4, 0x00020000);
  }
  __device__ __forceinline__ void issue(const float* obs, int n, const NetDims& nd, unsigned base, int tid) {
    const __amdgpu_buffer_rsrc_t rs = block(obs, n, nd.D);
#pragma unroll
    for (int i = 0; i < ITERS; ++i)
      v[i] = __builtin_bit_cast(float, __builtin_amdgcn_raw_buffer_load_b32(rs, slot_offset(base, i, nd.D, tid), 0, 0));
  }
  __device__ __forceinline__ void commit(float* dst, int tid) const {
    const int kk = tid & 63, w = (tid >> 6) - 1;
#pragma unroll
    for (int i = 0; i < ITERS; ++i) {
      const int r = w + 3 * i;
      if (r < 16) dst[r * LDH + kk] = v[i];
    }
  }
  __device__ __forceinline__ void copy_out(float* rb_obs, int n, int D, unsigned base, int tid) const {
    const __amdgpu_buffer_rsrc_t rs = block(rb_obs, n, D);
#pragma unroll
    for (int i = 0; i < ITERS; ++i)
      __builtin_amdgcn_raw_buffer_store_b32(__builtin_bit_cast(unsigned, v[i]), rs, slot_offset(base, i, D, tid), 0, 0);
  }
};

template <int CTRL>
__device__ __forceinline__ float dpp_quad_f(float v) {
  return __builtin_bit_cast(float, __builtin_amdgcn_update_dpp(0, __builtin_bit_cast(int, v), CTRL, 0xF, 0xF, true));
}
__device__ __forceinline__ float quad_sum_f(float v) {
  v += dpp_quad_f<0xB1>(v);
  v += dpp_quad_f<0x4E>(v);
  return v;
}

template <bool KEEP_JOINT>
__device__ __forceinline__ void fwd_args_pin_lean(FwdArgs& a) {
  a.mask = nullptr;
  a.uniforms = nullptr;
  a.given_actions = nullptr;
  a.deterministic = 0;
  a.act_f32 = nullptr;
  a.entropy = nullptr;
  a.logits = nullptr;
#ifndef PH_LEAN_PROF
  a.prof = nullptr;
#endif
  a.pos_env = nullptr;
  a.rec_mask = nullptr;
  if constexpr (!KEEP_JOINT) {
    a.joint = nullptr;
    a.joint_ll = nullptr;
  }
  a.env_mask = nullptr;
  a.host_done = nullptr;
  __builtin_assume(a.rb_obs != nullptr);
  __builtin_assume(a.rb_act != nullptr);
  __builtin_assume(a.rb_rew != nullptr);
  __builtin_assume(a.rb_es != nullptr);
  __builtin_assume(a.rb_val != nullptr);
  __builtin_assume(a.rb_logp != nullptr);
  __builtin_assume(a.es_in != nullptr);
}
bool fwd_args_lean(const FwdArgs& a, bool joint_ok = false) {
  static int enabled = -1;
  if (enabled < 0) {
    const char* e = getenv("PH_ROLLOUT_LEAN");
    enabled = (e && e[0] == '0') ? 0 : 1;
  }
#ifdef PH_LEAN_PROF
  constexpr bool lean_prof = true;
#else
  constexpr bool lean_prof = false;
#endif
  return enabled && !a.mask && !a.uniforms && !a.given_actions && !a.deterministic && !a.act_f32 && !a.entropy && !a.logits && (lean_prof || !a.prof) &&
         !a.pos_env && !a.rec_mask && (joint_ok || (!a.joint && !a.joint_ll)) && !a.env_mask && !a.host_done && a.rb_obs && a.rb_act && a.rb_rew &&
         a.rb_es && a.rb_val && a.rb_logp && a.es_in;
}

constexpr int ZS_FLOATS = 4 * 16 * 8;

template <bool VALU, int LEAN = 0>
__device__ __forceinline__ void policy_fwd16_body(const FwdArgs& a0, const ph_p2p* px = nullptr, int px_t = 0, int px_a_local = 0,
                                                  int agent = 0, const ScriptedSteps* sc = nullptr, int px_persistent = 0) {
  extern __shared__ __attribute__((aligned(16))) float smem[];
  constexpr int R = 16, NT = 256;
  const NetDims& nd = a0.nd;
  FwdArgs a = a0;
  if constexpr (LEAN == 1) fwd_args_pin_lean<false>(a);
  if constexpr (LEAN == 2) fwd_args_pin_lean<true>(a);
#ifdef PH_LEAN_PROF
  long long* const prof0 = a0.prof;
#else
  long long* const prof0 = LEAN ? nullptr : a0.prof;
#endif
  float* xs = smem;
  float* hs = xs + R * LDH;
  float* zs = hs + R * LDH;
  int* rowphys = (int*)(zs + ZS_FLOATS);
  float* upre = (float*)(rowphys + 16);
  unsigned long long** pxll = (unsigned long long**)(upre + 32);

  const int tid = threadIdx.x;
  const int wave = tid >> 6, lane = tid & 63, c = lane & 15, g = lane >> 4;
  const int net = blockIdx.y;
  const int row0 = blockIdx.x * R;
  const ph_layout& lay = nd.lay;
  const float* W1 = a.params + (net == 0 ? lay.pi_W1 : lay.vf_W1);
  const float* B1 = a.params + (net == 0 ? lay.pi_b1 : lay.vf_b1);
  const float* W2 = a.params + (net == 0 ? lay.pi_W2 : lay.vf_W2);
  const float* B2 = a.params + (net == 0 ? lay.pi_b2 : lay.vf_b2);
  const int nk = nd.L;

  PH_STAMP(a.prof, 0);
  if (tid < R) rowphys[tid] = (row0 + tid < a.n) ? row0 + tid : -1;
  constexpr bool PXH = LEAN != 0;
  const int pxw_h = (PXH && px) ? px->world : 0, pxc_h = (PXH && px) ? px->count : 0, pxr_h = (PXH && px) ? px->rank : 0;
  const int pxT_h = (PXH && px) ? px->T : 1, pxslots_h = (PXH && px) ? px->ll_slots : 1;
  unsigned long long* const ll_self_h = (PXH && px) ? px->ll[pxr_h] : nullptr;
  if (PXH && px && tid < pxw_h && tid < PH_MAX_RANKS) pxll[tid] = px->ll[tid];
#define pxw (PXH ? pxw_h : px->world)
#define pxc (PXH ? pxc_h : px->count)
#define pxr (PXH ? pxr_h : px->rank)
#define pxT (PXH ? pxT_h : px->T)
#define pxslots (PXH ? pxslots_h : px->ll_slots)
#define ll_self (PXH ? ll_self_h : px->ll[px->rank])
#define PXLL(p) (PXH ? pxll[p] : px->ll[p])
  float bw1[16], bw2[16], bwh[4];
  const int col = 16 * wave + c;
#pragma unroll
  for (int s = 0; s < 16; ++s) {
    const int k = g + 4 * s;
    bw1[s] = (k < nd.F) ? W1[k * HID + col] : 0.f;
    bw2[s] = W2[k * HID + col];
  }
#pragma unroll
  for (int s = 0; s < 4; ++s) {
    const int k = g + 4 * (4 * wave + s);
    bwh[s] = 0.f;
    if (net == 0) {
      if (c < nk) bwh[s] = a.params[lay.act_W + k * nk + c];
    } else if (c == 0) {
      bwh[s] = a.params[lay.val_W + k];
    }
  }
  const float bias1 = B1[col], bias2 = B2[col];
  float hbias = 0.f;
  if (wave == 0) {
    if (net == 0) hbias = (c < nk) ? a.params[lay.act_b + c] : 0.f;
    else hbias = (c == 0) ? a.params[lay.val_b] : 0.f;
  }
  XStage<R, NT> xr;
  lds_only_barrier();
  if (sc) a.obs = sc->obs_seq;
  xr.issue(rowphys, a.obs, nd, 0);
  const bool staged = sc != nullptr && nd.obs_kind == PH_SPACE_BOX;
  const bool copy_staged = staged && net == 1 && a.rb_obs && !a.pos_env && wave != 0;
  const unsigned roff = RowStage3::base_offset(row0, nd, tid);
  RowStage3 rows;
  if (copy_staged) rows.issue(a.obs, a0.n, nd, roff, tid);
  xr.commit(xs, rowphys, a.obs, nd, 0);
  vm_drain();
  if (copy_staged) rows.copy_out(a.rb_obs, a0.n, nd.D, roff, tid);
  lds_only_barrier();
  PH_STAMP(a.prof, 1);

  const int n_steps = sc ? sc->n_steps : 1;
  unsigned long long epoch_hi = 0ull;
  if (sc) {
    epoch_hi = a0.epoch ? (unsigned long long)(*a0.epoch) << 32 : 0ull;
    a.epoch = nullptr;
    a.counter = a0.counter + epoch_hi;
  }
  const unsigned long long px_epoch = (px && px_persistent) ? *px->epoch : 0ull;
  const bool draw_ahead = sc && net == 0 && !a.uniforms && !a.deterministic && !a.given_actions;
  auto draw_uniforms = [&](int t1) {
    if (lane < R && row0 + lane < a0.n)
      upre[(t1 & 1) * R + lane] = philox_uniform(a0.seed, a0.counter + (unsigned long long)t1 + epoch_hi, (uint32_t)(row0 + lane), 0u);
  };
  if (draw_ahead && wave == 1) draw_uniforms(0);

  auto product = [&](const float* A, const float (&bw)[16]) -> f32x4 {
    f32x4 e = {0.f, 0.f, 0.f, 0.f}, o = {0.f, 0.f, 0.f, 0.f};
    const float* ap = A + c * LDH + g;
    float av[16];
#pragma unroll
    for (int s = 0; s < 16; ++s) av[s] = ap[4 * s];
    __builtin_amdgcn_sched_barrier(0);
#pragma unroll
    for (int s = 0; s < 16; s += 2) {
      e = mma16<VALU>(av[s], bw[s], e, lane);
      o = mma16<VALU>(av[s + 1], bw[s + 1], o, lane);
    }
    return e + o;
  };

  for (int t = 0; t < n_steps; ++t) {
  long long* const pstep = (sc && t == 8) ? prof0 : nullptr;
  PH_STAMP(pstep, 8);
  if (t > 0) {
    const size_t row = (size_t)t * a0.n;
    a.obs = sc->obs_seq + row * nd.D;
    a.counter = a0.counter + (unsigned long long)t + epoch_hi;
    a.rb_obs = a0.rb_obs + row * nd.D;
    a.rb_act = a0.rb_act + row * nd.A;
    a.rb_rew = a0.rb_rew + row;
    a.rb_es = a0.rb_es + row;
    a.rb_val = a0.rb_val + row;
    a.rb_logp = a0.rb_logp + row;
    a.es_in = sc->done_seq + (row - a0.n);
    a.pending_reward = sc->rew_seq + (row - a0.n);
    a.prev_rew = a0.rb_rew + (row - a0.n);
    if constexpr (!LEAN) {
      a.mask = (sc->mask_seq && sc->mask_policy) ? sc->mask_seq + row * nd.L : nullptr;
      a.env_mask = (sc->mask_seq && sc->mask_env) ? sc->mask_seq + row * nd.L : nullptr;
    }
// ... 11 lines not shown
    lds_only_barrier();
  }
  PH_STAMP(pstep, 9);
  const bool more = t + 1 < n_steps;
  const float* const obs_next = sc ? sc->obs_seq + (size_t)(t + 1) * a0.n * nd.D : nullptr;

  const bool pre_ok = net == 1 && wave == 0 && lane < R && row0 + lane < a.n && !a.pos_env && a.rb_val;
  ValuePre vpre = {0.f, 0.f, 0.f, 0ull, 0ull, 0u, 0, 0};
  if (pre_ok) vpre = value_row_preload(a, row0 + lane);
  const bool copy_from_regs = net == 1 && a.rb_obs && !a.pos_env && nd.obs_kind == PH_SPACE_BOX;
  {
    const f32x4 z1 = product(xs, bw1);
#pragma unroll
    for (int r = 0; r < 4; ++r) hs[(4 * g + r) * LDH + col] = fast_tanh(z1[r] + bias1);
  }
  lds_only_barrier();
  PH_STAMP(a.prof, 3);
  PH_STAMP(pstep, 10);
  {
    const f32x4 z2 = product(hs, bw2);
#pragma unroll
    for (int r = 0; r < 4; ++r) xs[(4 * g + r) * LDH + col] = fast_tanh(z2[r] + bias2);
  }
  lds_only_barrier();
  PH_STAMP(a.prof, 5);
  PH_STAMP(pstep, 11);

  if (staged && net == 1 && more && wave != 0) rows.issue(obs_next, a0.n, nd, roff, tid);

  {
    if (wave == 0 && pre_ok) value_row_preload_words(a, row0 + lane, vpre);
    const float* ap = xs + c * LDH + g + 16 * wave;
    float av[4];
#pragma unroll
    for (int j = 0; j < 4; ++j) av[j] = ap[4 * j];
    f32x4 e = {0.f, 0.f, 0.f, 0.f}, o = {0.f, 0.f, 0.f, 0.f};
    e = mma16<VALU>(av[0], bwh[0], e, lane);
    o = mma16<VALU>(av[1], bwh[1], o, lane);
    e = mma16<VALU>(av[2], bwh[2], e, lane);
    o = mma16<VALU>(av[3], bwh[3], o, lane);
    const f32x4 zh = e + o;
    if (c < 8) {
#pragma unroll
      for (int r = 0; r < 4; ++r) zs[(wave * R + 4 * g + r) * 8 + c] = zh[r] + hbias;
    }
  }
  lds_only_barrier();
  PH_STAMP(pstep, 12);
  if (sc) vm_drain();
  if (staged && more && wave != 0) {
    if (net == 1) {
      rows.commit(xs, tid);
      if (copy_staged) rows.copy_out(a0.rb_obs + (size_t)(t + 1) * a0.n * nd.D, a0.n, nd.D, roff, tid);
    }
  }
  if (wave == 0) {
    PH_STAMP(pstep, 13);
    const int r = lane, grow = row0 + lane;
    if (r < R && grow < a.n) {
      float z[8];
      {
        float4 q[4][2];
#pragma unroll
        for (int w = 0; w < 4; ++w) {
          q[w][0] = *reinterpret_cast<const float4*>(zs + (w * R + r) * 8);
          q[w][1] = *reinterpret_cast<const float4*>(zs + (w * R + r) * 8 + 4);
        }
#pragma unroll
        for (int h = 0; h < 2; ++h) {
          z[4 * h + 0] = (q[0][h].x + q[1][h].x) + (q[2][h].x + q[3][h].x);
          z[4 * h + 1] = (q[0][h].y + q[1][h].y) + (q[2][h].y + q[3][h].y);
          z[4 * h + 2] = (q[0][h].z + q[1][h].z) + (q[2][h].z + q[3][h].z);
          z[4 * h + 3] = (q[0][h].w + q[1][h].w) + (q[2][h].w + q[3][h].w);
        }
      }
      if (net == 0) {
        const float* up = draw_ahead ? upre + (t & 1) * R + r : nullptr;
        const uint64_t ctr = fwd_counter(a);
        int act;
        switch (nk) {
          case 1: act = discrete8_row_tail<1>(a, nd, grow, z, ctr, up, pstep); break;
          case 2: act = discrete8_row_tail<2>(a, nd, grow, z, ctr, up, pstep); break;
          case 3: act = discrete8_row_tail<3>(a, nd, grow, z, ctr, up, pstep); break;
          case 4: act = discrete8_row_tail<4>(a, nd, grow, z, ctr, up, pstep); break;
          case 5: act = discrete8_row_tail<5>(a, nd, grow, z, ctr, up, pstep); break;
          case 6: act = discrete8_row_tail<6>(a, nd, grow, z, ctr, up, pstep); break;
          case 7: act = discrete8_row_tail<7>(a, nd, grow, z, ctr, up, pstep); break;
          default: act = discrete8_row_tail<8>(a, nd, grow, z, ctr, up, pstep); break;
        }
        if (px) {
          const int pt = px_t + t;
          const int slot = px_persistent ? p2p_persistent_slot(px_epoch, pxT, pt) : pt % pxslots;
          const size_t off = (size_t)slot * pxw * pxc + (size_t)(pxr * px_a_local + agent) * a.n + grow;
          const unsigned long long w =
              ((unsigned long long)p2p_stamp32(px_persistent ? px_epoch : *px->epoch, pxT, pt) << 32) | (unsigned long long)(unsigned)act;
          for (int p = 0; p < pxw; ++p)
            __hip_atomic_store(PXLL(p) + off, w, __ATOMIC_RELAXED, __HIP_MEMORY_SCOPE_SYSTEM);
        }
      } else {
        value_row_tail(a, grow, z[0], !a.pos_env && a.rb_val, vpre);
        if (sc && t == n_steps - 1) {
          float add = sc->rew_seq[(size_t)t * a0.n + grow];
          if (px_persistent && a0.joint) {
            FwdArgs b = a;
            b.joint_ll = ll_self + (size_t)p2p_persistent_slot(px_epoch, pxT, t) * pxw * pxc;
            b.ll_t = t;
// ... 2 lines not shown
            const int mine = ll_read(b, b.joint_ll + (size_t)a0.seat * a0.n + grow);
            const int theirs = ll_read(b, b.joint_ll + (size_t)p * a0.n + grow);
            add += joint_reward(mine, theirs, a0.bonus, a0.reward_rule);
          }
          a.rb_rew[grow] += add;
        }
      }
    }
  }
  PH_STAMP(pstep, 14);
  const bool stage_here = staged && net == 0 && more && wave != 0;
  if (stage_here) rows.issue(obs_next, a0.n, nd, roff, tid);
  if (draw_ahead && wave == 1 && more) draw_uniforms(t + 1);
  if (stage_here) {
    rows.commit(xs, tid);
    vm_drain();
  }
  if (copy_from_regs) {
    if (!staged) {
      const int kk = tid & 63;
#pragma unroll
      for (int i = 0; i < XStage<R, NT>::ITERS; ++i) {
        const int rr = (tid + NT * i) >> 6;
        if (kk < nd.D && row0 + rr < a.n) a.rb_obs[(size_t)(row0 + rr) * nd.D + kk] = xr.v[i];
      }
    }
  } else if (net == 1) {
    copy_obs_rows(a, row0, (a.n - row0 < R) ? a.n - row0 : R, nd.D);
  }
  PH_STAMP(a.prof, 7);
  PH_STAMP(pstep, 15);
  }
}

#undef pxw
#undef pxc
#undef pxr
#undef pxT
#undef pxslots
#undef ll_self
#undef PXLL

template <bool VALU, bool LEAN = false>
__global__ __launch_bounds__(256) void policy_fwd16_kernel(FwdArgs a) {
  policy_fwd16_body<VALU, LEAN ? 1 : 0>(a);
  if constexpr (!LEAN) {
    if (a.host_done) {
      __threadfence_system();
      __syncthreads();
      if (threadIdx.x == 0) __hip_atomic_store(a.host_done + blockIdx.y, a.host_seq, __ATOMIC_RELEASE, __HIP_MEMORY_SCOPE_SYSTEM);
    }
  }
}
template <bool VALU, bool LEAN>
__global__ __launch_bounds__(256) void policy_fwd16_rollout_kernel(FwdArgs a, ScriptedSteps sc) {
  policy_fwd16_body<VALU, LEAN ? 1 : 0>(a, nullptr, 0, 0, 0, &sc);
}
template <bool LEAN>
__global__ __launch_bounds__(256) void policy_fwd16_multi_kernel(FwdMulti m) {
  policy_fwd16_body<false, LEAN ? 2 : 0>(m.a[blockIdx.z], m.px.x, m.px.t, m.px.a_local, blockIdx.z);
}
template <bool LEAN>
__global__ __launch_bounds__(256, 3) void policy_fwd16_exchange_rollout_kernel(FwdMulti m, ScriptedMulti sm) {
  policy_fwd16_body<false, LEAN ? 2 : 0>(m.a[blockIdx.z], m.px.x, 0, m.px.a_local, blockIdx.z, &sm.sc[blockIdx.z], 1);
}

static size_t fwd16_lds_bytes() { return sizeof(float) * (size_t)(2 * 16 * LDH + ZS_FLOATS + 16 + 32) + sizeof(void*) * PH_MAX_RANKS; }

bool fwd16_eligible(const NetDims& nd, int n) {
  static int enabled = -1;
  if (enabled < 0) {
    const char* e = getenv("PH_FWD16");
    enabled = (e && e[0] == '0') ? 0 : 1;
  }
  return enabled && !nd.gauss && nd.nchunk == 1 && nd.A == 1 && nd.L <= 8 && n < 16384;
}

template <bool VALU>
static hipError_t launch_fwd16_variant(const FwdArgs& a, hipStream_t s) {
  const size_t lds = fwd16_lds_bytes();
  const bool general = VALU || !fwd_args_lean(a);
  const void* fn = general ? (const void*)policy_fwd16_kernel<VALU> : (const void*)policy_fwd16_kernel<false, true>;
  if (const hipError_t e = allow_dynamic_lds(fn, lds); e != hipSuccess) return e;
  if (general) hipLaunchKernelGGL((policy_fwd16_kernel<VALU>), dim3((a.n + 15) / 16, 2), dim3(256), lds, s, a);
  else hipLaunchKernelGGL((policy_fwd16_kernel<false, true>), dim3((a.n + 15) / 16, 2), dim3(256), lds, s, a);
  return hipGetLastError();
}

static size_t rollout_lds_bytes(int nwg_total) {
  const int cu = device_cu_count();
  return (cu > 0 && 2 * nwg_total <= cu) ? (size_t)81 * 1024 + 512 : fwd16_lds_bytes();
}
hipError_t launch_policy_fwd16_rollout(const FwdArgs& a, const ScriptedSteps& sc, int gemm_mode, hipStream_t s) {
  dim3 grid((a.n + 15) / 16, 2), block(256);
  const size_t lds = rollout_lds_bytes((int)(grid.x * grid.y));
  const int variant = gemm_mode == 1 ? 1 : ((fwd_args_lean(a) && !sc.mask_seq) ? 2 : 0);
  const void* fn = variant == 1 ? (const void*)policy_fwd16_rollout_kernel<true, false>
                                : (variant == 2 ? (const void*)policy_fwd16_rollout_kernel<false, true> : (const void*)policy_fwd16_rollout_kernel<false, false>);
  if (const hipError_t e = allow_dynamic_lds(fn, lds); e != hipSuccess) return e;
  if (variant == 1) hipLaunchKernelGGL((policy_fwd16_rollout_kernel<true, false>), grid, block, lds, s, a, sc);
  else if (variant == 2) hipLaunchKernelGGL((policy_fwd16_rollout_kernel<false, true>), grid, block, lds, s, a, sc);
  else hipLaunchKernelGGL((policy_fwd16_rollout_kernel<false, false>), grid, block, lds, s, a, sc);
  return hipGetLastError();
}

hipError_t exchange_rollout_blocks_per_cu(int* blocks_out) {
  const size_t lds = fwd16_lds_bytes();
  int api = 0;
  hipError_t e = hipOccupancyMaxActiveBlocksPerMultiprocessor(&api, (const void*)policy_fwd16_exchange_rollout_kernel<false>, 256, lds);
  if (e != hipSuccess) return e;
  const int by_lds = (int)((size_t)160 * 1024 / lds);
  int blocks = api < 8 ? api : 8;
  if (blocks > by_lds) blocks = by_lds;
  else if (blocks < by_lds && blocks > 1) blocks -= 1;
  *blocks_out = blocks < 1 ? 1 : blocks;
  return hipSuccess;
}

hipError_t launch_policy_fwd16_exchange_rollout(const FwdMulti& m, const ScriptedMulti& sm, int n_agents, hipStream_t s) {
  bool lean = true;
  for (int i = 0; i < n_agents; ++i) lean = lean && fwd_args_lean(m.a[i], true) && !sm.sc[i].mask_seq;
  const dim3 grid((m.a[0].n + 15) / 16, 2, n_agents);
  if (lean) hipLaunchKernelGGL(policy_fwd16_exchange_rollout_kernel<true>, grid, dim3(256), fwd16_lds_bytes(), s, m, sm);
  else hipLaunchKernelGGL(policy_fwd16_exchange_rollout_kernel<false>, grid, dim3(256), fwd16_lds_bytes(), s, m, sm);
  return hipGetLastError();
}

template <int CTRL>
__device__ __forceinline__ float dpp_f(float v) {
  return __builtin_bit_cast(float, __builtin_amdgcn_update_dpp(0, __builtin_bit_cast(int, v), CTRL, 0xF, 0xF, true));
}
template <bool MAX>
__device__ __forceinline__ float seg_scan32(float v, int k, int lo) {
  const int kr = k & 15;
#define PH_SCAN_STEP(D, CTRL)                                   \
  {                                                             \
    const float o = dpp_f<CTRL>(v);                             \
    const bool ok = kr >= (D) && k - (D) >= lo;                 \
    v = ok ? (MAX ? fmaxf(v, o) : v + o) : v;                   \
  }
  PH_SCAN_STEP(1, 0x111)
  PH_SCAN_STEP(2, 0x112)
  PH_SCAN_STEP(4, 0x114)
  PH_SCAN_STEP(8, 0x118)
#undef PH_SCAN_STEP
  const float o = dpp_f<0x142>(v);
  const bool ok = k >= 16 && lo <= 15;
  return ok ? (MAX ? fmaxf(v, o) : v + o) : v;
}
// ... 1036 lines not shown
```

### pantheonrl_amd/csrc/ph_ppo.hip

```cpp
#include "ph_launch.h"
#include "ph_split.h"
#include "ph_step.h"

namespace ph {


template <int N>
__device__ __forceinline__ float lds_colsum(const float* p, int stride, float s) {
#pragma unroll
  for (int r0 = 0; r0 < N; r0 += 16) {
    float t[16];
#pragma unroll
    for (int i = 0; i < 16; ++i) t[i] = p[(r0 + i) * stride];
    __builtin_amdgcn_sched_barrier(0);
#pragma unroll
    for (int i = 0; i < 16; ++i) s += t[i];
  }
  return s;
}
template <int N>
__device__ __forceinline__ float lds_coldot(const float* p, int stride, const float* q, int qstride, float s) {
#pragma unroll
  for (int r0 = 0; r0 < N; r0 += 16) {
    float t[16], u[16];
// ... 797 lines not shown
    s += __shfl_down(s, off, 64);
    q += __shfl_down(q, off, 64);
  }
  if (lane == 0) {
    sh[0][wave] = s;
    sh[1][wave] = q;
  }
  __syncthreads();
  if (tid == 0) {
    double ts = 0.0, tq = 0.0;
    for (int w = 0; w < ADV_THREADS / 64; ++w) {
      ts += sh[0][w];
      tq += sh[1][w];
    }
    a.partial[((size_t)mb * ADV_SPLIT + seg) * 2 + 0] = ts;
    a.partial[((size_t)mb * ADV_SPLIT + seg) * 2 + 1] = tq;
  }
}
__global__ void adv_finalize_kernel(AdvStatArgs a, int n_total) {
  const int mb = blockIdx.x * blockDim.x + threadIdx.x;
  if (mb >= n_total) return;
  const int k = mb % a.n_mb;
  const int start = k * a.batch;
  const int nb = (a.N - start < a.batch) ? a.N - start : a.batch;
  double ts = 0.0, tq = 0.0;
  for (int seg = 0; seg < ADV_SPLIT; ++seg) {
    ts += a.partial[((size_t)mb * ADV_SPLIT + seg) * 2 + 0];
    tq += a.partial[((size_t)mb * ADV_SPLIT + seg) * 2 + 1];
  }
  const double mean = ts / (double)nb;
  double var = (nb > 1) ? (tq - (double)nb * mean * mean) / (double)(nb - 1) : 0.0;
  if (var < 0.0) var = 0.0;
  a.out[2 * mb + 0] = (float)mean;
  a.out[2 * mb + 1] = (float)sqrt(var);
}
hipError_t launch_adv_stats(const AdvStatArgs& a, int n_total, hipStream_t s) {
  hipLaunchKernelGGL(adv_stats_kernel, dim3(n_total * ADV_SPLIT), dim3(ADV_THREADS), 0, s, a);
  hipLaunchKernelGGL(adv_finalize_kernel, dim3((n_total + 63) / 64), dim3(64), 0, s, a, n_total);
  return hipGetLastError();
}

constexpr int OP_ROWS = 32;
struct RowScalars {
  const float *adv, *logp, *act, *ret, *val;
  uint4* rowrec;
};
__global__ __launch_bounds__(256) void obs_planes_kernel(const float* __restrict__ obs, int n, int D, int F, int fold,
                                                         uint4* __restrict__ image, RowScalars rs) {
  __shared__ float xs[OP_ROWS][65];
  const int tid = threadIdx.x;
  const size_t row0 = (size_t)blockIdx.x * OP_ROWS;
  const int nrow = (row0 + OP_ROWS <= (size_t)n) ? OP_ROWS : (int)((size_t)n > row0 ? (size_t)n - row0 : 0);
  const float* src = obs + row0 * D;
  for (int e = tid; e < nrow * D; e += 256) {
    const int r = e / D, f = e - r * D;
    if (f < F) xs[r][f] = __builtin_nontemporal_load(src + e);
  }
  __syncthreads();
  const int r = tid >> 3, g = tid & 7;
  const size_t row = row0 + r;
  if (row > (size_t)n) return;
  if (rs.rowrec && row < (size_t)n && g < 2) {
    uint4 v = make_uint4(0u, 0u, 0u, 0u);
    if (g == 0) v = make_uint4(__float_as_uint(rs.adv[row]), __float_as_uint(rs.logp[row]), __float_as_uint(rs.act[row]), 0u);
    else v = make_uint4(__float_as_uint(rs.ret[row]), __float_as_uint(rs.val[row]), 0u, 0u);
    rs.rowrec[2 * row + g] = v;
  }
  typedef __bf16 bf8 __attribute__((ext_vector_type(8)));
  bf8 pl[3];
#pragma unroll
  for (int e = 0; e < 8; ++e) {
    const int f = 8 * g + e;
    float x = 0.f;
    if (row < (size_t)n) x = f < F ? xs[r][f] : ((fold && f == HID - 1) ? 1.f : 0.f);
    __bf16 h, m, l;
    split1(x, h, m, l);
    pl[0][e] = h;
    pl[1][e] = m;
    pl[2][e] = l;
  }
#pragma unroll
  for (int p = 0; p < 3; ++p) image[row * XIMG_ROW_U4 + p * 8 + g] = __builtin_bit_cast(uint4, pl[p]);
}
hipError_t launch_obs_planes(const float* obs, int n, int D, int F, int fold, uint4* image, const float* adv, const float* logp,
                             const float* act, const float* ret, const float* val, uint4* rowrec, hipStream_t s) {
  const size_t blocks = ((size_t)n + 1 + OP_ROWS - 1) / OP_ROWS;
  RowScalars rs{adv, logp, act, ret, val, (adv && logp && act && ret && val) ? rowrec : nullptr};
  hipLaunchKernelGGL(obs_planes_kernel, dim3((unsigned)blocks), dim3(256), 0, s, obs, n, D, F, fold, image, rs);
  return hipGetLastError();
}

template <int VEC>
__global__ __launch_bounds__(RED_PARAMS * 4) void ppo_reduce_kernel(ReduceArgs a) {
  __shared__ float lds_union[4 * RED_PARAMS];
  static_assert(4 * RED_PARAMS >= 32 * NSTATP + NSTATP || 4 * RED_PARAMS >= 32 * NSTATP, "statistics scratch within the slab scratch");
  float (*gsum)[RED_PARAMS] = reinterpret_cast<float (*)[RED_PARAMS]>(lds_union);
  float (*part)[NSTATP] = reinterpret_cast<float (*)[NSTATP]>(lds_union);
  __shared__ float means[NSTATP];
  const int tid = threadIdx.x;
  if (*a.stop_flag != 0) {
    if (blockIdx.x == 0 && tid < PH_NSTAT && a.stats_out) a.stats_out[tid] = 0.f;
    if (blockIdx.x == 0 && tid == 0) {
      a.scalars[1] = 0.f;
      a.scalars[2] = 0.f;
    }
    return;
  }
  if (blockIdx.x == gridDim.x - 1) {
    (void)reduce_statistics(a, part, means, true);
    return;
  }
  const int dst = reduce_dst(a, blockIdx.x);
  const float g = reduce_positions<VEC>(a, gsum, dst, blockIdx.x);
  if (tid < 64) {
    if (dst >= 0) a.grad[dst] = g;
    float q = g * g;
    for (int off = 32; off > 0; off >>= 1) q += __shfl_down(q, off, 64);
    if (tid == 0) a.blocksq[blockIdx.x] = q;
  }
}

template <int VEC>
__global__ __launch_bounds__(RED_PARAMS * 4) void ppo_step_kernel(StepArgs s) {
  __shared__ float gsum[4][RED_PARAMS];
  __shared__ float part[32][NSTATP];
  __shared__ float means[NSTATP];
  const int nblk = gridDim.x - 1;
  const int stopped = *s.r.stop_flag;
  const unsigned tag = *s.gen + 1u;
  const int step_new = *s.ad.step + 1;
  const unsigned err = *s.sweep_error;
  step_body<VEC>(s, blockIdx.x, nblk, tag, step_new, gsum, part, means, nullptr, stopped, err);
}

int reduce_blocks(int slab_len) { return (slab_len + RED_PARAMS - 1) / RED_PARAMS; }
static int reduce_vec(int slab_len, int exclusive) { return (slab_len % 4 == 0 && exclusive) ? 4 : (slab_len % 2 == 0 ? 2 : 1); }
bool step_fused_fits(int nblk, int slab_len, int num_cu) {
  if (nblk + 1 > 64 * 16) return false;
  static int per_cu[3] = {-1, -1, -1};
  const int vec = reduce_vec(slab_len, 1);
  int& v = per_cu[vec == 4 ? 2 : vec - 1];
// ... 137 lines not shown
```

### pantheonrl_amd/ppo.py

```python
from __future__ import annotations

import ctypes as C
import os
import io
import json
import time
import zipfile
from collections import deque
from typing import Sequence, Any, Dict, Optional, Tuple

import numpy as np
import torch as th

from . import _native as nat
from . import spaces as sp
from .logger import Logger, configure_logger

HID = nat.PH_HIDDEN


def _require_cuda(device) -> th.device:
    dev = th.device("cuda" if device in (None, "auto") else device)
    if dev.type != "cuda":
        raise nat.NativeError(
# ... 59 lines not shown
        o, a = _f32_dev(obs, dev, (E, D)), _f32_dev(action, dev, (E, A))
        s, v, lp = _f32_dev(episode_start, dev, (E,)), _f32_dev(value, dev, (E,)), _f32_dev(log_prob, dev, (E,))
        self._bind()
        nat.check(self.ctx.lib.ph_buffer_add(self.ctx.handle, C.byref(self.spec), C.byref(self._c), self.pos,
                                             o.data_ptr(), a.data_ptr(), s.data_ptr(), v.data_ptr(), lp.data_ptr()))
        self.pos += 1
        r = np.asarray(reward.detach().cpu() if isinstance(reward, th.Tensor) else reward, dtype=np.float32)
        if np.any(r != 0):
            self.add_reward(r)
        self.full = self.pos == self.buffer_size

    def add_reward(self, reward, env_mask=None, pos: Optional[int] = None) -> None:
        row = (self.pos - 1) % self.buffer_size if pos is None else pos
        if (env_mask is None and self.n_envs == 1 and isinstance(reward, np.ndarray) and reward.size == 1):
            reward = float(reward.reshape(-1)[0])
        if env_mask is None and isinstance(reward, (int, float, np.floating, np.integer)):
            self._bind()
            nat.check(self.ctx.lib.ph_buffer_add_reward_const(self.ctx.handle, C.byref(self._c), row, float(reward)))
            return
        r = _f32_dev(np.broadcast_to(np.asarray(reward, np.float32), (self.n_envs,))
                     if not isinstance(reward, th.Tensor) else reward, self.device, (self.n_envs,))
        m = None
        if env_mask is not None:
            m = th.as_tensor(env_mask).to(device=self.device, dtype=th.uint8).contiguous()
        self._bind()
        nat.check(self.ctx.lib.ph_buffer_add_reward(self.ctx.handle, C.byref(self._c), row, r.data_ptr(), nat.ptr(m)))

    def compute_returns_and_advantage(self, last_values, dones) -> None:
        E, dev = self.n_envs, self.device
        lv = _f32_dev(last_values, dev, (E,))
        dn = _f32_dev(np.broadcast_to(np.asarray(dones, np.float32), (E,)) if not isinstance(dones, th.Tensor)
                      else dones, dev, (E,))
        self._bind()
        nat.check(self.ctx.lib.ph_gae(self.ctx.handle, C.byref(self._c), lv.data_ptr(), dn.data_ptr(), self.gamma,
                                      self.gae_lambda, int(self.gae_mode)))

    def _bind(self) -> None:
        self.ctx.set_stream(_raw_stream(self.device))

    def c_struct(self) -> nat.PhRollout:
        return self._c

    def c_ref(self):
        ref = self.__dict__.get("_c_byref")
        if ref is None:
            ref = self._c_byref = C.byref(self._c)
        return ref

    def add_reward_scalar(self, reward: float) -> None:
        self._bind()
        rc = self.ctx.lib.ph_buffer_add_reward_const(self.ctx.handle, self.c_ref(), (self.pos - 1) % self.buffer_size, reward)
        if rc:
            nat.check(rc)

    def host(self) -> Dict[str, np.ndarray]:
        return {k: getattr(self, k).detach().cpu().numpy() for k in (
            "observations", "actions", "rewards", "episode_starts", "values", "log_probs", "advantages", "returns")}


_SD = (("mlp_extractor.policy_net.0", "pi_W1", "pi_b1"), ("mlp_extractor.policy_net.2", "pi_W2", "pi_b2"),
       ("mlp_extractor.value_net.0", "vf_W1", "vf_b1"), ("mlp_extractor.value_net.2", "vf_W2", "vf_b2"),
       ("action_net", "act_W", "act_b"), ("value_net", "val_W", "val_b"))


class _HostStep:

    def __init__(self, pol, obs_shape):
        lay = pol.layout
        n = int(np.prod(obs_shape)) // lay.D
        if n * lay.D != int(np.prod(obs_shape)) or n <= 0:
            raise ValueError(f"observation rows of shape {tuple(obs_shape)} do not hold whole rows of {lay.D} values")
        self.n = n
        self.rows = np.empty((n, lay.D), np.float32)
        self.rows_nd = self.rows.reshape(obs_shape)
        self.acts = np.empty((n, lay.A), np.int32)
        self.acts_shaped = self.acts.reshape((-1,) + tuple(pol.action_space.shape))
        self.vals, self.logp, self.es = np.empty((n, 1), np.float32), np.empty((n,), np.float32), np.empty((n,), np.float32)
        self.rows_ptr, self.acts_ptr = self.rows.ctypes.data, self.acts.ctypes.data
        self.vals_ptr, self.logp_ptr, self.es_ptr = self.vals.ctypes.data, self.logp.ctypes.data, self.es.ctypes.data
        self.spec_ref = C.byref(pol.spec)
        self.params, self.params_ptr = pol.params, pol.params.data_ptr()


class ActorCriticPolicy:

    host_step_path = True
    fused_mlp_kernels = True

    def __init__(self, observation_space, action_space, lr: float = 3e-4, device="cuda",
                 ortho_init: bool = True, seed: Optional[int] = None, sampling_stream: int = 0):
        if type(action_space).__name__ == "Box" and not getattr(self, "gaussian_head", False):
            raise UnsupportedPolicyConfig(f"{type(self).__name__} is written for the categorical heads (Discrete / MultiDiscrete "
                                          "actions); Box action spaces run on PPO's GaussianActorCriticPolicy (DiagGaussian head)")
        self.device = _require_cuda(device)
        self.observation_space, self.action_space = observation_space, action_space
        self.spec = sp.make_spec(observation_space, action_space)
        self.layout = nat.layout_of(self.spec)
        self.ctx = nat.Context(self.device.index)
        self.gemm_mode = int(os.environ.get("PH_GEMM_MODE", "2"))
        lay = self.layout
        self.params = th.zeros(lay.P, dtype=th.float32, device=self.device)
        self.adam_m = th.zeros_like(self.params)
        self.adam_v = th.zeros_like(self.params)
        self.opt_step = th.zeros(1, dtype=th.int32, device=self.device)
        self.lr = float(lr(1.0)) if callable(lr) else float(lr)
        self._seed = int(seed) if seed is not None else int(np.random.randint(0, 2 ** 31 - 1))
# ... 764 lines not shown
```

Before: 121.6 million agent-steps/s.

## Hand off bf16 observation planes and row records from rollout and GAE to gradient

The scripted rollout kernel now writes the split bf16 observation planes straight into the context's gradient image while it stages observations. GAE now emits the per-row scalar record table as it computes advantages. The gradient setup then skips the separate obs_planes pass whenever validity tracking shows both products are current. This removes a full re-read and re-split of the rollout buffer per update, at the cost of extra stores in the rollout kernel and state-tracking that must be invalidated correctly on any intervening call.

```diff
diff --git a/include/pantheon_hip.h b/include/pantheon_hip.h
--- a/include/pantheon_hip.h
+++ b/include/pantheon_hip.h
@@ -84,6 +84,10 @@
 int ph_rng_epoch_advance(ph_ctx *ctx);
 int ph_debug_set_profile_buffer(ph_ctx *ctx, long long *stamps_dev);
 int ph_debug_weight_image_mismatches(ph_ctx *ctx, const ph_spec *spec, const float *params, int *mismatches);
+int ph_ctx_invalidate_grad_pack(ph_ctx *ctx);
+int ph_debug_grad_pack_check(ph_ctx *ctx, const ph_spec *spec, const ph_rollout *rb, int *state_out, int *image_mismatches,
+                             int *table_mismatches);
+int ph_debug_grad_pack_copy(ph_ctx *ctx, int rows, void *image_host, void *table_host);
 int ph_set_exclusive_device(ph_ctx *ctx, int exclusive);
 int ph_ctx_step_errors(ph_ctx *ctx, unsigned int *count_out );
 int ph_timer_start(ph_ctx *ctx);
diff --git a/pantheonrl_amd/_native.py b/pantheonrl_amd/_native.py
--- a/pantheonrl_amd/_native.py
+++ b/pantheonrl_amd/_native.py
@@ -236,6 +236,9 @@
     "ph_set_exclusive_device": [_vp, _i],
     "ph_ctx_step_errors": [_vp, C.POINTER(C.c_uint)],
     "ph_debug_weight_image_mismatches": [_vp, C.POINTER(PhSpec), _vp, C.POINTER(C.c_int)],
+    "ph_ctx_invalidate_grad_pack": [_vp],
+    "ph_debug_grad_pack_check": [_vp, C.POINTER(PhSpec), C.POINTER(PhRollout), C.POINTER(C.c_int), C.POINTER(C.c_int), C.POINTER(C.c_int)],
+    "ph_debug_grad_pack_copy": [_vp, _i, _vp, _vp],
     "ph_timer_start": [_vp],
     "ph_timer_stop": [_vp, C.POINTER(C.c_float)],
     "ph_layout_of": [C.POINTER(PhSpec), C.POINTER(PhLayout)],
@@ -456,6 +459,9 @@
     def set_joint_reward_rule(self, rule: str) -> None:
         check(self.lib.ph_ctx_set_joint_reward_rule(self.handle, {"match": 0, "rps": 1}[rule]))
 
+    def invalidate_grad_pack(self) -> None:
+        check(self.lib.ph_ctx_invalidate_grad_pack(self.handle))
+
     def step_errors(self) -> int:
         n = C.c_uint(0)
         check(self.lib.ph_ctx_step_errors(self.handle, C.byref(n)))
diff --git a/pantheonrl_amd/csrc/ph_abi.hip b/pantheonrl_amd/csrc/ph_abi.hip
--- a/pantheonrl_amd/csrc/ph_abi.hip
+++ b/pantheonrl_amd/csrc/ph_abi.hip
@@ -138,6 +138,16 @@
   size_t rec_cap = 0;
   uint4* rowrec = nullptr;
   size_t rowrec_cap = 0;
+  struct GradPack {
+    const float* obs = nullptr;
+    int T = 0, E = 0, D = 0, F = 0, fold = 0, spec_id = 0;
+    const float* adv = nullptr;
+    int rec_T = 0, rec_E = 0;
+    bool planes = false, records = false;
+    const float* want_adv = nullptr;
+    int want_T = 0, want_E = 0;
+  } pack;
+  size_t ximg_zero_rows = ~(size_t)0;
   unsigned long long* step_words = nullptr;
   size_t step_words_cap = 0;
   unsigned int* step_gen = nullptr;
@@ -187,8 +197,12 @@
 struct DevGuard {
   int prev = -1;
   bool switched = false;
-  explicit DevGuard(const ph_ctx* ctx) {
+  explicit DevGuard(const ph_ctx* ctx, bool keeps_pack = false) {
     if (!ctx) return;
+    if (!keeps_pack) {
+      ph_ctx::GradPack& pk = const_cast<ph_ctx*>(ctx)->pack;
+      pk.planes = pk.records = false;
+    }
     if (hipGetDevice(&prev) == hipSuccess && prev != ctx->device) switched = hipSetDevice(ctx->device) == hipSuccess;
   }
   ~DevGuard() {
@@ -534,6 +548,57 @@
 }
 int hip_rc(hipError_t e, const char* what) { return e == hipSuccess ? 0 : fail_hip(what, e); }
 
+bool pack_handoff_enabled() {
+  const char* e = getenv("PH_GRAD_PACK_HANDOFF");
+  return !(e && e[0] == '0');
+}
+bool pack_check_enabled() {
+  const char* e = getenv("PH_GRAD_PACK_CHECK");
+  return e && e[0] == '1';
+}
+bool pack_has_planes(const ph_ctx* ctx, const ph::NetDims& nd, const ph_rollout* rb) {
+  const ph_ctx::GradPack& pk = ctx->pack;
+  const size_t rows = (size_t)rb->T * rb->E;
+  return pk.planes && pk.obs == rb->observations && pk.T == rb->T && pk.E == rb->E && pk.D == nd.D && pk.F == nd.F &&
+         pk.fold == (ph::grad_fast_fold(nd) ? 1 : 0) && pk.spec_id == nd.spec_id && ctx->ximg && (rows + 1) * ph::XIMG_ROW_U4 <= ctx->ximg_cap &&
+         ctx->ximg_zero_rows == rows;
+}
+bool pack_has_records(const ph_ctx* ctx, const ph_rollout* rb) {
+  const ph_ctx::GradPack& pk = ctx->pack;
+  return pk.records && pk.adv == rb->advantages && pk.rec_T == rb->T && pk.rec_E == rb->E && ctx->rowrec &&
+         2 * (size_t)rb->T * rb->E <= ctx->rowrec_cap;
+}
+int pack_mismatches(ph_ctx* ctx, const ph::NetDims& nd, const ph_rollout* rb, bool planes, bool records, int* image_bad, int* table_bad) {
+  *image_bad = *table_bad = -1;
+  if (!planes && !records) return 0;
+  if (ctx->capturing) return fail("the gradient pack's check synchronises: not inside graph capture");
+  const size_t rows = (size_t)rb->T * rb->E, n_img = (rows + 1) * ph::XIMG_ROW_U4, n_tab = 2 * rows;
+  if ((planes && (!ctx->ximg || n_img > ctx->ximg_cap)) || (records && (!ctx->rowrec || n_tab > ctx->rowrec_cap)))
+    return fail("the gradient pack's check: the context holds no image / table of this buffer's size");
+  uint4 *img = nullptr, *tab = nullptr;
+  int* cnt = nullptr;
+  int host[2] = {0, 0};
+  hipError_t e = hipMalloc((void**)&img, n_img * sizeof(uint4));
+  if (e == hipSuccess) e = hipMalloc((void**)&tab, n_tab * sizeof(uint4));
+  if (e == hipSuccess) e = hipMalloc((void**)&cnt, 2 * sizeof(int));
+  hipStream_t s = ctx->stream;
+  if (e == hipSuccess) e = hipMemsetAsync(cnt, 0, 2 * sizeof(int), s);
+  if (e == hipSuccess)
+    e = ph::launch_obs_planes(rb->observations, (int)rows, nd.D, nd.F, ph::grad_fast_fold(nd) ? 1 : 0, img, rb->advantages, rb->log_probs,
+                              rb->actions, rb->returns, rb->values, tab, s);
+  if (e == hipSuccess && planes) e = ph::launch_grad_pack_check(ctx->ximg, img, n_img, cnt, s);
+  if (e == hipSuccess && records) e = ph::launch_grad_pack_check(ctx->rowrec, tab, n_tab, cnt + 1, s);
+  if (e == hipSuccess) e = hipMemcpyAsync(host, cnt, 2 * sizeof(int), hipMemcpyDeviceToHost, s);
+  if (e == hipSuccess) e = hipStreamSynchronize(s);
+  if (img) (void)hipFree(img);
+  if (tab) (void)hipFree(tab);
+  if (cnt) (void)hipFree(cnt);
+  if (e != hipSuccess) return fail_hip("the gradient pack's check", e);
+  if (planes) *image_bad = host[0];
+  if (records) *table_bad = host[1];
+  return 0;
+}
+
 }
 
 extern "C" {
@@ -618,14 +683,21 @@
 }
 
 int ph_ctx_set_stream(ph_ctx* ctx, void* hip_stream) {
-  DevGuard dev_guard(ctx);
-  if (!ctx) return fail("null ctx");
+  DevGuard dev_guard(ctx, true);
+  if (!ctx) return fail("null ctx");
+  if (ctx->stream != (hipStream_t)hip_stream) ctx->pack.planes = ctx->pack.records = false;
   ctx->stream = (hipStream_t)hip_stream;
   return 0;
 }
 
+int ph_ctx_invalidate_grad_pack(ph_ctx* ctx) {
+  DevGuard dev_guard(ctx);
+  if (!ctx) return fail("null ctx");
+  return 0;
+}
+
 int ph_ctx_sync(ph_ctx* ctx) {
-  DevGuard dev_guard(ctx);
+  DevGuard dev_guard(ctx, true);
   if (!ctx) return fail("null ctx");
   PH_HIP(hipStreamSynchronize(ctx->stream));
   return 0;
@@ -666,13 +738,13 @@
 }
 
 int ph_ctx_set_rng_epoch(ph_ctx* ctx, unsigned long long* epoch_dev) {
-  DevGuard dev_guard(ctx);
+  DevGuard dev_guard(ctx, true);
   if (!ctx) return fail("null ctx");
   ctx->rng_epoch = epoch_dev;
   return 0;
 }
 int ph_rng_epoch_advance(ph_ctx* ctx) {
-  DevGuard dev_guard(ctx);
+  DevGuard dev_guard(ctx, true);
   if (!ctx) return fail("null ctx");
   if (!ctx->rng_epoch) return fail("ph_rng_epoch_advance: no epoch word attached");
   PH_HIP(ph::launch_epoch_advance(ctx->rng_epoch, ctx->stream));
@@ -680,14 +752,14 @@
 }
 
 int ph_debug_set_profile_buffer(ph_ctx* ctx, long long* stamps_dev) {
-  DevGuard dev_guard(ctx);
+  DevGuard dev_guard(ctx, true);
   if (!ctx) return fail("null ctx");
   ctx->prof = stamps_dev;
   return 0;
 }
 
 int ph_debug_weight_image_mismatches(ph_ctx* ctx, const ph_spec* spec, const float* params, int* mismatches_host) {
-  DevGuard dev_guard(ctx);
+  DevGuard dev_guard(ctx, true);
   if (!ctx || !params || !mismatches_host) return fail("ph_debug_weight_image_mismatches: null argument");
   ph::NetDims nd;
   if (resolve(ctx, spec, &nd)) return 1;
@@ -703,6 +775,35 @@
   return 0;
 }
 
+int ph_debug_grad_pack_check(ph_ctx* ctx, const ph_spec* spec, const ph_rollout* rb, int* state_out, int* image_mismatches_host,
+                             int* table_mismatches_host) {
+  DevGuard dev_guard(ctx, true);
+  if (!ctx || !state_out || !image_mismatches_host || !table_mismatches_host) return fail("ph_debug_grad_pack_check: null argument");
+  if (check_rb(rb)) return 1;
+  ph::NetDims nd;
+  if (resolve(ctx, spec, &nd)) return 1;
+  const bool planes = pack_has_planes(ctx, nd, rb), records = pack_has_records(ctx, rb);
+  *state_out = (planes ? 1 : 0) | (records ? 2 : 0);
+  return pack_mismatches(ctx, nd, rb, planes, records, image_mismatches_host, table_mismatches_host);
+}
+
+int ph_debug_grad_pack_copy(ph_ctx* ctx, int rows, void* image_host, void* table_host) {
+  DevGuard dev_guard(ctx, true);
+  if (!ctx || rows <= 0) return fail("ph_debug_grad_pack_copy: null ctx / no rows");
+  if (ctx->capturing) return fail("ph_debug_grad_pack_copy synchronises: not inside graph capture");
+  const size_t n_img = ((size_t)rows + 1) * ph::XIMG_ROW_U4, n_tab = 2 * (size_t)rows;
+  if (image_host) {
+    if (!ctx->ximg || n_img > ctx->ximg_cap) return fail("ph_debug_grad_pack_copy: the context's plane image is smaller than that");
+    PH_HIP(hipMemcpyAsync(image_host, ctx->ximg, n_img * sizeof(uint4), hipMemcpyDeviceToHost, ctx->stream));
+  }
+  if (table_host) {
+    if (!ctx->rowrec || n_tab > ctx->rowrec_cap) return fail("ph_debug_grad_pack_copy: the context's per-row table is smaller than that");
+    PH_HIP(hipMemcpyAsync(table_host, ctx->rowrec, n_tab * sizeof(uint4), hipMemcpyDeviceToHost, ctx->stream));
+  }
+  PH_HIP(hipStreamSynchronize(ctx->stream));
+  return 0;
+}
+
 int ph_set_exclusive_device(ph_ctx* ctx, int exclusive) {
   if (!ctx) return fail("null ctx");
   ctx->exclusive = exclusive != 0;
@@ -710,7 +811,7 @@
 }
 
 int ph_ctx_step_errors(ph_ctx* ctx, unsigned int* count_out) {
-  DevGuard dev_guard(ctx);
+  DevGuard dev_guard(ctx, true);
   if (!ctx || !count_out) return fail("ph_ctx_step_errors: null argument");
   *count_out = 0u;
   if (!ctx->step_gen) return 0;
@@ -720,13 +821,13 @@
 }
 
 int ph_timer_start(ph_ctx* ctx) {
-  DevGuard dev_guard(ctx);
+  DevGuard dev_guard(ctx, true);
   if (!ctx) return fail("null ctx");
   PH_HIP(hipEventRecord(ctx->ev0, ctx->stream));
   return 0;
 }
 int ph_timer_stop(ph_ctx* ctx, float* ms_out) {
-  DevGuard dev_guard(ctx);
+  DevGuard dev_guard(ctx, true);
   if (!ctx || !ms_out) return fail("null ctx/ms_out");
   PH_HIP(hipEventRecord(ctx->ev1, ctx->stream));
   PH_HIP(hipEventSynchronize(ctx->ev1));
@@ -807,7 +908,7 @@
 
 int ph_buffer_add_reward(ph_ctx* ctx, const ph_rollout* rb, int pos, const float* reward,
                          const unsigned char* env_mask) {
-  DevGuard dev_guard(ctx);
+  DevGuard dev_guard(ctx, true);
   if (!ctx) return fail("null ctx");
   if (check_rb(rb)) return 1;
   if (pos < 0 || pos >= rb->T) return fail("ph_buffer_add_reward: pos out of range");
@@ -817,7 +918,7 @@
 }
 
 int ph_buffer_add_reward_const(ph_ctx* ctx, const ph_rollout* rb, int pos, float reward) {
-  DevGuard dev_guard(ctx);
+  DevGuard dev_guard(ctx, true);
   if (!ctx) return fail("null ctx");
   if (check_rb(rb)) return 1;
   if (pos < 0 || pos >= rb->T) return fail("ph_buffer_add_reward_const: pos out of range");
@@ -827,7 +928,7 @@
 
 int ph_buffer_add_reward_joint(ph_ctx* ctx, const ph_rollout* rb, int pos, const float* base_reward,
                                const int* joint_actions, int n_seats, int seat, const int* partner_seat, float bonus) {
-  DevGuard dev_guard(ctx);
+  DevGuard dev_guard(ctx, true);
   if (!ctx) return fail("null ctx");
   if (check_rb(rb)) return 1;
   if (pos < 0 || pos >= rb->T) return fail("ph_buffer_add_reward_joint: pos out of range");
@@ -997,13 +1098,29 @@
 
 int ph_gae(ph_ctx* ctx, const ph_rollout* rb, const float* last_values, const float* dones, double gamma,
            double gae_lambda, int mode) {
-  DevGuard dev_guard(ctx);
+  DevGuard dev_guard(ctx, true);
   if (!ctx) return fail("null ctx");
   if (check_rb(rb)) return 1;
   if (!last_values || !dones) return fail("ph_gae: null last_values/dones");
   if (mode < 0 || mode > 2) return fail("ph_gae: mode must be 0, 1 or 2");
+  ph_ctx::GradPack& pk = ctx->pack;
+  const size_t rows = (size_t)rb->T * rb->E;
+  pk.records = false;
+  bool with_records = pack_handoff_enabled() && ((pk.planes && pk.obs == rb->observations && pk.T == rb->T && pk.E == rb->E) ||
+                                                 (pk.want_adv == rb->advantages && pk.want_T == rb->T && pk.want_E == rb->E));
+  if (with_records && 2 * rows > ctx->rowrec_cap) {
+    if (ctx->capturing) with_records = false;
+    else if (ensure(ctx, ctx->rowrec, ctx->rowrec_cap, 2 * rows)) return 1;
+  }
   PH_HIP(ph::launch_gae(rb->rewards, rb->values, rb->episode_starts, last_values, dones, rb->advantages, rb->returns,
-                        rb->T, rb->E, gamma, gae_lambda, mode, ctx->stream));
+                        rb->T, rb->E, gamma, gae_lambda, mode, ctx->stream, with_records ? ctx->rowrec : nullptr, rb->log_probs,
+                        rb->actions));
+  if (with_records) {
+    pk.adv = rb->advantages;
+    pk.rec_T = rb->T;
+    pk.rec_E = rb->E;
+    pk.records = true;
+  }
   return 0;
 }
 
@@ -1106,7 +1223,7 @@
                         const float* done_seq, int n, int n_steps, const float* episode_start0, unsigned long long seed,
                         unsigned long long counter0, int* actions_i32, float* values, float* log_probs, const ph_rollout* rb,
                         int pos0, int gemm_mode) {
-  DevGuard dev_guard(ctx);
+  DevGuard dev_guard(ctx, true);
   if (!ctx) return fail("null ctx");
   if (!params || !obs_seq || !rew_seq || !done_seq || !episode_start0) return fail("ph_scripted_rollout: null argument");
   if ((uintptr_t)params % 16 != 0) return fail("ph_scripted_rollout: params must be 16-byte aligned");
@@ -1127,7 +1244,40 @@
   sc.rew_seq = rew_seq;
   sc.done_seq = done_seq;
   sc.mask_seq = nullptr;
+  sc.mask_policy = sc.mask_env = 0;
+  sc.ximg = nullptr;
+  sc.ximg_fold = 0;
+  ph_ctx::GradPack& pk = ctx->pack;
+  pk.planes = pk.records = false;
+  const bool planes = pack_handoff_enabled() && gemm_mode == 2 && a.nd.split_kind == 1 && a.nd.obs_kind == PH_SPACE_BOX && pos0 == 0 &&
+                      n_steps == rb->T;
+  const size_t rows = (size_t)rb->T * rb->E;
+  if (planes) {
+    if ((rows + 1) * ph::XIMG_ROW_U4 > ctx->ximg_cap) {
+      if (ctx->capturing) return fail("the plane image would grow inside graph capture: run the same call once outside capture first");
+      if (ensure(ctx, ctx->ximg, ctx->ximg_cap, (rows + 1) * ph::XIMG_ROW_U4)) return 1;
+      ctx->ximg_zero_rows = ~(size_t)0;
+    }
+    if (ctx->ximg_zero_rows != rows) {
+      if (ctx->capturing) return fail("the plane image changes its row count inside graph capture: run the same call once outside capture first");
+      PH_HIP(hipMemsetAsync(ctx->ximg + rows * ph::XIMG_ROW_U4, 0, ph::XIMG_ROW_U4 * sizeof(uint4), ctx->stream));
+      ctx->ximg_zero_rows = rows;
+    }
+    sc.ximg = reinterpret_cast<unsigned short*>(ctx->ximg);
+    sc.ximg_fold = ph::grad_fast_fold(a.nd) ? 1 : 0;
+  }
   PH_HIP(ph::launch_policy_fwd16_rollout(a, sc, gemm_mode, ctx->stream));
+  if (planes) {
+    pk.obs = rb->observations;
+    pk.adv = nullptr;
+    pk.T = rb->T;
+    pk.E = rb->E;
+    pk.D = a.nd.D;
+    pk.F = a.nd.F;
+    pk.fold = sc.ximg_fold;
+    pk.spec_id = a.nd.spec_id;
+    pk.planes = true;
+  }
   return 0;
 }
 
@@ -2056,6 +2206,14 @@
   if (nd.split != 1) return 0;
   const size_t rows = (size_t)rb->T * rb->E;
   const size_t need_img = (rows + 1) * ph::XIMG_ROW_U4;
+  ph_ctx::GradPack& pk = ctx->pack;
+  const bool have_planes = pack_handoff_enabled() && pack_has_planes(ctx, nd, rb);
+  const bool have_records = pack_handoff_enabled() && pack_has_records(ctx, rb);
+  pk.planes = pk.records = false;
+  pk.want_adv = rb->advantages;
+  pk.want_T = rb->T;
+  pk.want_E = rb->E;
+  if (need_img > ctx->ximg_cap) ctx->ximg_zero_rows = ~(size_t)0;
   if (ensure(ctx, ctx->ximg, ctx->ximg_cap, need_img)) return 1;
   if (ensure(ctx, ctx->rowrec, ctx->rowrec_cap, 2 * rows)) return 1;
   if (n_rec > ctx->rec_cap) {
@@ -2064,8 +2222,19 @@
     if (ensure(ctx, ctx->rec_vf, c2, n_rec)) return 1;
     ctx->rec_cap = n_rec;
   }
-  PH_HIP(ph::launch_obs_planes(rb->observations, (int)rows, nd.D, nd.F, ph::grad_fast_fold(nd) ? 1 : 0, ctx->ximg, rb->advantages,
-                               rb->log_probs, rb->actions, rb->returns, rb->values, ctx->rowrec, ctx->stream));
+  if (!have_planes || !have_records) {
+    PH_HIP(ph::launch_obs_planes(rb->observations, (int)rows, nd.D, nd.F, ph::grad_fast_fold(nd) ? 1 : 0, have_planes ? nullptr : ctx->ximg,
+                                 rb->advantages, rb->log_probs, rb->actions, rb->returns, rb->values, have_records ? nullptr : ctx->rowrec,
+                                 ctx->stream));
+    if (!have_planes) ctx->ximg_zero_rows = rows;
+  }
+  if ((have_planes || have_records) && pack_check_enabled()) {
+    int image_bad = 0, table_bad = 0;
+    if (pack_mismatches(ctx, nd, rb, have_planes, have_records, &image_bad, &table_bad)) return 1;
+    if (image_bad > 0 || table_bad > 0)
+      return fail("gradient pack hand-off: " + std::to_string(image_bad < 0 ? 0 : image_bad) + " words of the plane image and " + std::to_string(table_bad < 0 ? 0 : table_bad) +
+                  " words of the per-row table differ from obs_planes_kernel's");
+  }
   return 0;
 }
 void fill_adv_records(ph::AdvStatArgs& aa, const ph_ctx* ctx, const ph::NetDims& nd, const ph_rollout* rb) {
@@ -2325,14 +2494,14 @@
 int ph_ppo_train(ph_ctx* ctx, const ph_spec* spec, const ph_opt_state* opt, const ph_rollout* rb,
                  const ph_ppo_hyper* hp, int n_epochs, int batch_size, const int* perms,
                  unsigned long long perm_seed, float* stats, int gemm_mode) {
-  DevGuard dev_guard(ctx);
+  DevGuard dev_guard(ctx, true);
   return train_run("ph_ppo_train", ctx, spec, opt, rb, hp, n_epochs, batch_size, perms, perm_seed, stats, gemm_mode, nullptr);
 }
 
 int ph_adap_train(ph_ctx* ctx, const ph_spec* spec, const ph_opt_state* opt, const ph_rollout* rb,
                   const ph_ppo_hyper* hp, int n_epochs, int batch_size, const int* perms,
                   unsigned long long perm_seed, float* stats, int gemm_mode, const ph_adap_loss* adap) {
-  DevGuard dev_guard(ctx);
+  DevGuard dev_guard(ctx, true);
   if (!adap) return fail("ph_adap_train: null context-term description");
   return train_run("ph_adap_train", ctx, spec, opt, rb, hp, n_epochs, batch_size, perms, perm_seed, stats, gemm_mode, adap);
 }
@@ -2379,14 +2548,14 @@
 int ph_ppo_minibatch_grad(ph_ctx* ctx, const ph_spec* spec, const float* params, const ph_rollout* rb,
                           const ph_ppo_hyper* hp, const int* indices, int nb, float* grad_out, float* stats_out,
                           int gemm_mode) {
-  DevGuard dev_guard(ctx);
+  DevGuard dev_guard(ctx, true);
   return minibatch_grad_run("ph_ppo_minibatch_grad", ctx, spec, params, rb, hp, indices, nb, grad_out, stats_out, gemm_mode, nullptr);
 }
 
 int ph_adap_minibatch_grad(ph_ctx* ctx, const ph_spec* spec, const float* params, const ph_rollout* rb,
                            const ph_ppo_hyper* hp, const int* indices, int nb, float* grad_out, float* stats_out,
                            int gemm_mode, const ph_adap_loss* adap) {
-  DevGuard dev_guard(ctx);
+  DevGuard dev_guard(ctx, true);
   if (!adap) return fail("ph_adap_minibatch_grad: null context-term description");
   return minibatch_grad_run("ph_adap_minibatch_grad", ctx, spec, params, rb, hp, indices, nb, grad_out, stats_out, gemm_mode, adap);
 }
diff --git a/pantheonrl_amd/csrc/ph_gae.hip b/pantheonrl_amd/csrc/ph_gae.hip
--- a/pantheonrl_amd/csrc/ph_gae.hip
+++ b/pantheonrl_amd/csrc/ph_gae.hip
@@ -1,11 +1,21 @@
 #include "ph_launch.h"
 
 namespace ph {
+
+struct GaeRecords {
+  uint4* rowrec;
+  const float* logp;
+  const float* act;
+};
+__device__ __forceinline__ void gae_record(const GaeRecords& rec, size_t o, float adv, float ret, float val) {
+  rec.rowrec[2 * o] = make_uint4(__float_as_uint(adv), __float_as_uint(rec.logp[o]), __float_as_uint(rec.act[o]), 0u);
+  rec.rowrec[2 * o + 1] = make_uint4(__float_as_uint(ret), __float_as_uint(val), 0u, 0u);
+}
 
 __global__ __launch_bounds__(64) void gae_serial_kernel(const float* __restrict__ rew, const float* __restrict__ val,
                                                         const float* __restrict__ es, const float* __restrict__ last_values,
                                                         const float* __restrict__ dones, float* __restrict__ adv,
-                                                        float* __restrict__ ret, int T, int E, float g, float gl) {
+                                                        float* __restrict__ ret, int T, int E, float g, float gl, GaeRecords rec) {
 #pragma clang fp contract(off)
   const int e = blockIdx.x * blockDim.x + threadIdx.x;
   if (e >= E) return;
@@ -27,8 +37,10 @@
       const size_t o = (size_t)(t - u) * E + e;
       const float delta = (r[u] + (g * nv) * nnt) - v[u];
       last = delta + ((gl * nnt) * last);
+      const float rt = last + v[u];
       adv[o] = last;
-      ret[o] = last + v[u];
+      ret[o] = rt;
+      if (rec.rowrec) gae_record(rec, o, last, rt, v[u]);
       nv = v[u];
       nnt = 1.0f - s[u];
     }
@@ -38,8 +50,10 @@
     const float r = rew[o], v = val[o], s = es[o];
     const float delta = (r + (g * nv) * nnt) - v;
     last = delta + ((gl * nnt) * last);
+    const float rt = last + v;
     adv[o] = last;
-    ret[o] = last + v;
+    ret[o] = rt;
+    if (rec.rowrec) gae_record(rec, o, last, rt, v);
     nv = v;
     nnt = 1.0f - s;
   }
@@ -54,7 +68,7 @@
                                                         const float* __restrict__ last_values,
                                                         const float* __restrict__ dones, float* __restrict__ adv,
                                                         float* __restrict__ ret, int T, int E, int NCH, float g,
-                                                        float gl) {
+                                                        float gl, GaeRecords rec) {
   extern __shared__ __attribute__((aligned(16))) float sm[];
   float* sS = sm;
   float* sP = sm + NCH * EB;
@@ -138,8 +152,10 @@
         if (t >= 0) {
           const size_t o = (size_t)t * E + e;
           const float A = a[k] + cp[k] * Ain;
+          const float R = A + vv[k];
           gae_st(adv + o, A);
-          gae_st(ret + o, A + vv[k]);
+          gae_st(ret + o, R);
+          if (rec.rowrec) gae_record(rec, o, A, R, vv[k]);
         }
       }
     }
@@ -148,7 +164,8 @@
 
 template <int LC, int EB>
 static hipError_t launch_scan(const float* rew, const float* val, const float* es, const float* lv, const float* dn,
-                              float* adv, float* ret, int T, int E, float g, float gl, hipStream_t s, int max_chunks = 1024 / EB) {
+                              float* adv, float* ret, int T, int E, float g, float gl, hipStream_t s, const GaeRecords& rec,
+                              int max_chunks = 1024 / EB) {
   int NCH = (T + LC - 1) / LC;
   int maxch = max_chunks < 1024 / EB ? max_chunks : 1024 / EB;
   static int nch_env = -1;
@@ -160,18 +177,20 @@
   if (NCH > maxch) NCH = maxch;
   dim3 grid((E + EB - 1) / EB), block(NCH * EB);
   const size_t lds = sizeof(float) * (2 * NCH * EB + EB);
-  hipLaunchKernelGGL((gae_scan_kernel<LC, EB>), grid, block, lds, s, rew, val, es, lv, dn, adv, ret, T, E, NCH, g, gl);
+  hipLaunchKernelGGL((gae_scan_kernel<LC, EB>), grid, block, lds, s, rew, val, es, lv, dn, adv, ret, T, E, NCH, g, gl, rec);
   return hipGetLastError();
 }
 
 hipError_t launch_gae(const float* rew, const float* val, const float* es, const float* lv, const float* dn, float* adv,
-                      float* ret, int T, int E, double gamma, double lam, int mode, hipStream_t s) {
+                      float* ret, int T, int E, double gamma, double lam, int mode, hipStream_t s, uint4* rowrec, const float* logp,
+                      const float* act) {
+  const GaeRecords rec{(logp && act) ? rowrec : nullptr, logp, act};
   const float g = (float)gamma;
   const float gl = (float)(gamma * lam);
   if (mode == 0) mode = 2;
   if (mode == 1) {
     hipLaunchKernelGGL(gae_serial_kernel, dim3((E + 63) / 64), dim3(64), 0, s, rew, val, es, lv, dn, adv, ret, T, E, g,
-                       gl);
+                       gl, rec);
     return hipGetLastError();
   }
   static int lc_env = -1;
@@ -179,12 +198,12 @@
     const char* e = getenv("PH_GAE_LC");
     lc_env = e ? atoi(e) : 0;
   }
-  if (lc_env == 8) return launch_scan<8, 32>(rew, val, es, lv, dn, adv, ret, T, E, g, gl, s);
-  if (lc_env == 16) return launch_scan<16, 32>(rew, val, es, lv, dn, adv, ret, T, E, g, gl, s);
-  if (lc_env == 32) return launch_scan<32, 32>(rew, val, es, lv, dn, adv, ret, T, E, g, gl, s);
-  if (T <= 256) return launch_scan<8, 32>(rew, val, es, lv, dn, adv, ret, T, E, g, gl, s);
-  if (E >= 16384) return launch_scan<16, 64>(rew, val, es, lv, dn, adv, ret, T, E, g, gl, s, 16);
-  return launch_scan<16, 32>(rew, val, es, lv, dn, adv, ret, T, E, g, gl, s, 8);
+  if (lc_env == 8) return launch_scan<8, 32>(rew, val, es, lv, dn, adv, ret, T, E, g, gl, s, rec);
+  if (lc_env == 16) return launch_scan<16, 32>(rew, val, es, lv, dn, adv, ret, T, E, g, gl, s, rec);
+  if (lc_env == 32) return launch_scan<32, 32>(rew, val, es, lv, dn, adv, ret, T, E, g, gl, s, rec);
+  if (T <= 256) return launch_scan<8, 32>(rew, val, es, lv, dn, adv, ret, T, E, g, gl, s, rec);
+  if (E >= 16384) return launch_scan<16, 64>(rew, val, es, lv, dn, adv, ret, T, E, g, gl, s, rec, 16);
+  return launch_scan<16, 32>(rew, val, es, lv, dn, adv, ret, T, E, g, gl, s, rec, 8);
 }
 
 __global__ void buffer_add_kernel(float* __restrict__ d_obs, float* __restrict__ d_act, float* __restrict__ d_rew,
diff --git a/pantheonrl_amd/csrc/ph_launch.h b/pantheonrl_amd/csrc/ph_launch.h
--- a/pantheonrl_amd/csrc/ph_launch.h
+++ b/pantheonrl_amd/csrc/ph_launch.h
@@ -78,6 +78,8 @@
   const float* done_seq;
   const unsigned char* mask_seq;
   int mask_policy, mask_env;
+  unsigned short* ximg;
+  int ximg_fold;
 };
 
 constexpr int MAX_LOCAL_AGENTS = 4;
@@ -239,7 +241,8 @@
 hipError_t launch_policy_fwd_multi(const FwdMulti& m, int n_agents, hipStream_t s);
 hipError_t launch_fix_illegal(int* actions, const unsigned char* mask, int n, int L, hipStream_t s);
 hipError_t launch_gae(const float* rew, const float* val, const float* es, const float* lv, const float* dn, float* adv,
-                      float* ret, int T, int E, double gamma, double lam, int mode, hipStream_t s);
+                      float* ret, int T, int E, double gamma, double lam, int mode, hipStream_t s, uint4* rowrec = nullptr,
+                      const float* logp = nullptr, const float* act = nullptr);
 hipError_t launch_buffer_add(float* d_obs, float* d_act, float* d_rew, float* d_es, float* d_val, float* d_lp,
                              const float* obs, const float* act, const float* es, const float* val, const float* lp,
                              int E, int D, int A, hipStream_t s);
@@ -409,6 +412,7 @@
 constexpr int XIMG_ROW_U4 = 24;
 hipError_t launch_obs_planes(const float* obs, int n, int D, int F, int fold, uint4* image, const float* adv, const float* logp,
                              const float* act, const float* ret, const float* val, uint4* rowrec, hipStream_t s);
+hipError_t launch_grad_pack_check(const uint4* have, const uint4* want, size_t n_u4, int* mismatches, hipStream_t s);
 hipError_t launch_ppo_reduce(const ReduceArgs& a, hipStream_t s);
 int reduce_blocks(int slab_len);
 bool step_fused_fits(int nblk, int slab_len, int num_cu);
diff --git a/pantheonrl_amd/csrc/ph_policy.hip b/pantheonrl_amd/csrc/ph_policy.hip
--- a/pantheonrl_amd/csrc/ph_policy.hip
+++ b/pantheonrl_amd/csrc/ph_policy.hip
@@ -3,6 +3,7 @@
 #include "ph_rowtail.h"
 #include "ph_liar_group.h"
 #include "ph_pool.h"
+#include "ph_split.h"
 
 namespace ph {
 
@@ -167,6 +168,23 @@
 #pragma unroll
     for (int i = 0; i < ITERS; ++i)
       __builtin_amdgcn_raw_buffer_store_b32(__builtin_bit_cast(unsigned, v[i]), rs, slot_offset(base, i, D, tid), 0, 0);
+  }
+  __device__ __forceinline__ static unsigned plane_base_offset(int row0, int tid) {
+    const int kk = tid & 63, w = (tid >> 6) - 1;
+    return w >= 0 ? (unsigned)(row0 + w) * (unsigned)(XIMG_ROW_U4 * 16) + 2u * (unsigned)kk : NONE;
+  }
+  __device__ __forceinline__ void planes_out(unsigned short* img_blk, int n, unsigned pbase, int fold, int tid) const {
+    const __amdgpu_buffer_rsrc_t rs = __builtin_amdgcn_make_buffer_rsrc(img_blk, 0, n * XIMG_ROW_U4 * 16, 0x00020000);
+    const bool one = fold && (tid & 63) == HID - 1;
+#pragma unroll
+    for (int i = 0; i < ITERS; ++i) {
+      const unsigned off = (i == 5 && (tid >> 6) != 1) ? NONE : pbase + (unsigned)(3 * i) * (unsigned)(XIMG_ROW_U4 * 16);
+      __bf16 h, m, l;
+      split1(one ? 1.f : v[i], h, m, l);
+      __builtin_amdgcn_raw_buffer_store_b16(__builtin_bit_cast(unsigned short, h), rs, off, 0, 0);
+      __builtin_amdgcn_raw_buffer_store_b16(__builtin_bit_cast(unsigned short, m), rs, off + 128u, 0, 0);
+      __builtin_amdgcn_raw_buffer_store_b16(__builtin_bit_cast(unsigned short, l), rs, off + 256u, 0, 0);
+    }
   }
 };
 
@@ -226,7 +244,7 @@
 
 constexpr int ZS_FLOATS = 4 * 16 * 8;
 
-template <bool VALU, int LEAN = 0>
+template <bool VALU, int LEAN = 0, bool PLANES = false>
 __device__ __forceinline__ void policy_fwd16_body(const FwdArgs& a0, const ph_p2p* px = nullptr, int px_t = 0, int px_a_local = 0,
                                                   int agent = 0, const ScriptedSteps* sc = nullptr, int px_persistent = 0) {
   extern __shared__ __attribute__((aligned(16))) float smem[];
@@ -308,6 +326,10 @@
   xr.commit(xs, rowphys, a.obs, nd, 0);
   vm_drain();
   if (copy_staged) rows.copy_out(a.rb_obs, a0.n, nd.D, roff, tid);
+  const unsigned poff = RowStage3::plane_base_offset(row0, tid);
+  if constexpr (PLANES) {
+    if (copy_staged) rows.planes_out(sc->ximg, a0.n, poff, sc->ximg_fold, tid);
+  }
   lds_only_barrier();
   PH_STAMP(a.prof, 1);
 
@@ -425,6 +447,9 @@
     if (net == 1) {
       rows.commit(xs, tid);
       if (copy_staged) rows.copy_out(a0.rb_obs + (size_t)(t + 1) * a0.n * nd.D, a0.n, nd.D, roff, tid);
+      if constexpr (PLANES) {
+        if (copy_staged) rows.planes_out(sc->ximg + (size_t)(t + 1) * a0.n * (XIMG_ROW_U4 * 8), a0.n, poff, sc->ximg_fold, tid);
+      }
     }
   }
   if (wave == 0) {
@@ -533,9 +558,9 @@
     }
   }
 }
-template <bool VALU, bool LEAN>
+template <bool VALU, bool LEAN, bool PLANES = false>
 __global__ __launch_bounds__(256) void policy_fwd16_rollout_kernel(FwdArgs a, ScriptedSteps sc) {
-  policy_fwd16_body<VALU, LEAN ? 1 : 0>(a, nullptr, 0, 0, 0, &sc);
+  policy_fwd16_body<VALU, LEAN ? 1 : 0, PLANES>(a, nullptr, 0, 0, 0, &sc);
 }
 template <bool LEAN>
 __global__ __launch_bounds__(256) void policy_fwd16_multi_kernel(FwdMulti m) {
@@ -576,6 +601,14 @@
   dim3 grid((a.n + 15) / 16, 2), block(256);
   const size_t lds = rollout_lds_bytes((int)(grid.x * grid.y));
   const int variant = gemm_mode == 1 ? 1 : ((fwd_args_lean(a) && !sc.mask_seq) ? 2 : 0);
+  if (sc.ximg) {
+    if (variant == 1 || a.nd.obs_kind != PH_SPACE_BOX || !a.rb_obs || a.pos_env) return hipErrorInvalidValue;
+    const void* fp = variant == 2 ? (const void*)policy_fwd16_rollout_kernel<false, true, true> : (const void*)policy_fwd16_rollout_kernel<false, false, true>;
+    if (const hipError_t e = allow_dynamic_lds(fp, lds); e != hipSuccess) return e;
+    if (variant == 2) hipLaunchKernelGGL((policy_fwd16_rollout_kernel<false, true, true>), grid, block, lds, s, a, sc);
+    else hipLaunchKernelGGL((policy_fwd16_rollout_kernel<false, false, true>), grid, block, lds, s, a, sc);
+    return hipGetLastError();
+  }
   const void* fn = variant == 1 ? (const void*)policy_fwd16_rollout_kernel<true, false>
                                 : (variant == 2 ? (const void*)policy_fwd16_rollout_kernel<false, true> : (const void*)policy_fwd16_rollout_kernel<false, false>);
   if (const hipError_t e = allow_dynamic_lds(fn, lds); e != hipSuccess) return e;
diff --git a/pantheonrl_amd/csrc/ph_ppo.hip b/pantheonrl_amd/csrc/ph_ppo.hip
--- a/pantheonrl_amd/csrc/ph_ppo.hip
+++ b/pantheonrl_amd/csrc/ph_ppo.hip
@@ -873,9 +873,11 @@
   const size_t row0 = (size_t)blockIdx.x * OP_ROWS;
   const int nrow = (row0 + OP_ROWS <= (size_t)n) ? OP_ROWS : (int)((size_t)n > row0 ? (size_t)n - row0 : 0);
   const float* src = obs + row0 * D;
-  for (int e = tid; e < nrow * D; e += 256) {
-    const int r = e / D, f = e - r * D;
-    if (f < F) xs[r][f] = __builtin_nontemporal_load(src + e);
+  if (image) {
+    for (int e = tid; e < nrow * D; e += 256) {
+      const int r = e / D, f = e - r * D;
+      if (f < F) xs[r][f] = __builtin_nontemporal_load(src + e);
+    }
   }
   __syncthreads();
   const int r = tid >> 3, g = tid & 7;
@@ -887,6 +889,7 @@
     else v = make_uint4(__float_as_uint(rs.ret[row]), __float_as_uint(rs.val[row]), 0u, 0u);
     rs.rowrec[2 * row + g] = v;
   }
+  if (!image) return;
   typedef __bf16 bf8 __attribute__((ext_vector_type(8)));
   bf8 pl[3];
 #pragma unroll
@@ -908,6 +911,22 @@
   const size_t blocks = ((size_t)n + 1 + OP_ROWS - 1) / OP_ROWS;
   RowScalars rs{adv, logp, act, ret, val, (adv && logp && act && ret && val) ? rowrec : nullptr};
   hipLaunchKernelGGL(obs_planes_kernel, dim3((unsigned)blocks), dim3(256), 0, s, obs, n, D, F, fold, image, rs);
+  return hipGetLastError();
+}
+__global__ __launch_bounds__(256) void grad_pack_check_kernel(const uint4* __restrict__ have, const uint4* __restrict__ want, size_t n_u4,
+                                                              int* mismatches) {
+  int bad = 0;
+  for (size_t i = (size_t)blockIdx.x * 256 + threadIdx.x; i < n_u4; i += (size_t)gridDim.x * 256) {
+    const uint4 a = have[i], b = want[i];
+    bad += (a.x != b.x) + (a.y != b.y) + (a.z != b.z) + (a.w != b.w);
+  }
+  if (bad) atomicAdd(mismatches, bad);
+}
+hipError_t launch_grad_pack_check(const uint4* have, const uint4* want, size_t n_u4, int* mismatches, hipStream_t s) {
+  size_t blocks = (n_u4 + 255) / 256;
+  if (blocks > 4096) blocks = 4096;
+  if (blocks < 1) blocks = 1;
+  hipLaunchKernelGGL(grad_pack_check_kernel, dim3((unsigned)blocks), dim3(256), 0, s, have, want, n_u4, mismatches);
   return hipGetLastError();
 }
 
diff --git a/pantheonrl_amd/ppo.py b/pantheonrl_amd/ppo.py
--- a/pantheonrl_amd/ppo.py
+++ b/pantheonrl_amd/ppo.py
@@ -135,6 +135,9 @@
         rc = self.ctx.lib.ph_buffer_add_reward_const(self.ctx.handle, self.c_ref(), (self.pos - 1) % self.buffer_size, reward)
         if rc:
             nat.check(rc)
+
+    def invalidate_grad_pack(self) -> None:
+        self.ctx.invalidate_grad_pack()
 
     def host(self) -> Dict[str, np.ndarray]:
         return {k: getattr(self, k).detach().cpu().numpy() for k in (
```

Result: slower. 120.2 million agent-steps/s (-1.2%).
